# DonggeunYu/Text2Speech

Measured on AMD Instinct MI355X. Metric: WaveGlow forward audio samples/sec (batch 8x16000 per GPU), higher is better.
Workload: dtype bf16x3 (split-bf16 products, f32 accumulate); 1 GPU; WaveGlow forward, batch 8 x 16000 samples per GPU, 12 flows, n_group 8, WN 8 layers x 512 channels (reference waveglow/config.json); per_gpu_batch=8, segment_length=16000, mode=forward, parallelism=replicas, no collective

## Files before the change

include/t2s_hip.h:

```cpp
#ifndef T2S_HIP_H
#define T2S_HIP_H
#include <stddef.h>
#ifdef __cplusplus
extern "C" {
#endif

#define T2S_OK 0
#define T2S_EINVAL (-1)
#define T2S_EHIP (-2)

#define T2S_PERM_NONE 0
#define T2S_PERM_GATE 1
#define T2S_PERM_PAIR8 2
#define T2S_ACT_NONE 0
#define T2S_ACT_RELU 1
#define T2S_ACT_TANH 2

int t2s_abi_version(void);
int t2s_operand_format(void);
int t2s_sizeof_taco_decoder(void);
int t2s_sizeof_taco_bptt(void);
const char* t2s_error_string(int code);
const char* t2s_last_hip_error(void);

int t2s_plane_rows(int L, int halo);
int t2s_padded_rows(int rows);

int t2s_pack_conv_weight(const float* v, const float* g, int g_is_scale, const float* bias_in, int O, int Cin, int Kt,
                         int perm, int C_gate, int row_off, int Mpad, int koff, int Cin_pad, void* A_hi, void* A_lo,
                         float* bias_out, int bias_accumulate, void* stream);

typedef struct t2s_pack_job {
    const float *v, *g, *bias_in, *bias_in2;
    void *A_hi, *A_lo;
    float* bias_out;
    long row_start;
    long O, Cin, Kt, perm, C_gate, Mpad, koff, Cin_pad, row_off, g_is_scale;
    float* scale_out;
} t2s_pack_job;
int t2s_pack_conv_weight_table(const t2s_pack_job* jobs, int n_jobs, long total_groups, void* stream);

int t2s_weightnorm_small(const float* v, const float* g, int O, int K, float* w, void* stream);

int t2s_wg_upsample_squeeze(const float* mel, const float* W, const float* bias, int B, int n_mel, int frames,
                            int ksize, int stride, int n_group, int L, int Lp, int halo, void* S_hi, void* S_lo,
                            void* stream);

int t2s_wg_audio_squeeze(float* audio, float* z, int B, int T, int n_group, int L, int unsqueeze, void* stream);

int t2s_wg_convinv(float* z, const float* W, int B, int n_group, int c_off, int n_rem, int L, void* stream);

int t2s_small_logdet_inv(const float* W, int n, float scale, float* logdet_out, float* inv_out, void* stream);

typedef struct t2s_small_mat_job { const float* W; float* logdet_out; float* inv_out; long n; } t2s_small_mat_job;
int t2s_small_logdet_inv_batch(const t2s_small_mat_job* jobs, int n_jobs, float scale, void* stream);
int t2s_small_logdet_inv_batch_host(const t2s_small_mat_job* host_jobs, int n_jobs, float scale, void* stream);

int t2s_wg_start(const float* z, const float* w, const float* bias, int B, int n_group, int c_off, int n_half, int C,
                 int L, int Lp, int halo, void* X_hi, void* X_lo, void* stream);

int t2s_wg_in_cond_gate(const void* A_hi, const void* A_lo, const float* bias, const void* X_hi, const void* X_lo,
                        const void* S_hi, const void* S_lo, void* acts_hi, void* acts_lo, int B, int C, int n_cond,
                        int taps, int dilation, int L, int Lp, int halo, int Mpad, void* stream);

int t2s_wg_res_skip(const void* A_hi, const void* A_lo, const float* bias, const void* acts_hi, const void* acts_lo,
                    void* X_hi, void* X_lo, float* skip, int B, int C, int n_res, int skip_init, int L, int Lp,
                    int halo, int Mpad, void* stream);

int t2s_wg_end_affine(const float* skip, const float* w_end, const float* b_end, float* z, float* log_s,
                      float* wn_out, int B, int n_group, int c_off, int n_half, int C, int L, int Lp, int halo, int reverse, void* stream);

typedef struct t2s_endfold_job {
    const float *w_end, *v_skip, *scale, *b_skip;
    void* fold_A;
    float* bes;
    long nj, C;
} t2s_endfold_job;
int t2s_wg_endfold_weights(const t2s_endfold_job* jobs, int n_jobs, int C, void* stream);
int t2s_wg_gate_tile_rows(int B, int C, int L);
int t2s_wg_gate_fold_slots(int B, int C, int L);
int t2s_wg_in_cond_gate_fold(const void* A_hi, const void* A_lo, const float* bias, const void* X_hi, const void* X_lo,
                             const void* S_hi, const void* S_lo, void* acts_hi, void* acts_lo, const void* fold_A,
                             float* fold_acc, int fold_init, int B, int C, int n_cond, int taps, int dilation, int L,
                             int Lp, int halo, int Mpad, void* stream);
int t2s_wg_start_window(const float* z, const float* w, const float* bias, int B, int n_group, int c_off, int n_half, int C,
                        int L, int Lp, int halo, void* X_hi, void* X_lo, int taps, int win_chunks, void* W_hi, void* W_lo,
                        void* stream);
int t2s_wg_startfold_weights(const float* v_in, const float* g_in, const float* w_start, const float* b_start, int C, int n_half,
                             int taps, int Mpad, int win_chunks, void* A_hi, void* A_lo, void* stream);
int t2s_wg_in_win_gate_fold(const void* A_hi, const void* A_lo, const float* bias, const void* W_hi, const void* W_lo,
                            const void* S_hi, const void* S_lo, void* acts_hi, void* acts_lo, const void* fold_A,
                            float* fold_acc, int fold_init, int B, int C, int n_cond, int win_chunks, int L, int Lp, int halo,
                            int Mpad, void* stream);
int t2s_wg_upsample_basis(const float* W, const float* bias, int n_mel, int ksize, int stride, int n_group, int Lp, int halo,
                          void* U_hi, void* U_lo, void* stream);
int t2s_wg_compose_cond(const float* tmp, const float* bias_in, int rows, int Mpad, int P, int K2, long ld, void* A2_hi,
                        void* A2_lo, float* bias_out, void* stream);
int t2s_wg_melwin_planes(const float* mel, int B, int n_mel, int frames, int nlag, int Fp, void* M_hi, void* M_lo, void* stream);
int t2s_wg_in_melwin_gate_fold(const void* A_hi, const void* A_lo, const void* A2_hi, const void* A2_lo, const float* bias,
                               const void* X_hi, const void* X_lo, const void* M_hi, const void* M_lo, void* acts_hi,
                               void* acts_lo, const void* fold_A, float* fold_acc, int fold_init, int B, int C, int K2,
                               int taps, int dilation, int L, int Lp, int halo, int Mpad, int P, int Fp, void* stream);
int t2s_wg_res_only(const void* A_hi, const void* A_lo, const float* bias, const void* acts_hi, const void* acts_lo,
                    void* X_hi, void* X_lo, int B, int C, int L, int Lp, int halo, int Mpad, int pair8, void* stream);
int t2s_wg_res_only_start(const void* A_hi, const void* A_lo, const float* bias, const void* acts_hi, const void* acts_lo,
                          const float* z, const float* w_start, const float* b_start, int n_group, int c_off, int n_half,
                          void* X_hi, void* X_lo, int B, int C, int L, int Lp, int halo, int Mpad, void* stream);
int t2s_pack_conv_weight_table_h16(const t2s_pack_job* jobs, int n_jobs, long total_groups, void* stream);
int t2s_wg_endfold_weights_h16(const t2s_endfold_job* jobs, int n_jobs, int C, void* stream);
int t2s_wg_upsample_squeeze_h16(const float* mel, const float* W, const float* bias, int B, int n_mel, int frames,
                                int ksize, int stride, int n_group, int L, int Lp, int halo, void* S_hi, void* S_lo,
                                void* stream);
int t2s_wg_start_h16(const float* z, const float* w, const float* bias, int B, int n_group, int c_off, int n_half, int C,
                     int L, int Lp, int halo, void* X_hi, void* X_lo, void* stream);
int t2s_wg_in_cond_gate_fold_h16(const void* A_hi, const void* A_lo, const float* bias, const void* X_hi, const void* X_lo,
                                 const void* S_hi, const void* S_lo, void* acts_hi, void* acts_lo, const void* fold_A,
                                 float* fold_acc, int fold_init, int B, int C, int n_cond, int taps, int dilation, int L,
                                 int Lp, int halo, int Mpad, void* stream);
int t2s_wg_res_only_h16(const void* A_hi, const void* A_lo, const float* bias, const void* acts_hi, const void* acts_lo,
                        void* X_hi, void* X_lo, int B, int C, int L, int Lp, int halo, int Mpad, int pair8, void* stream);
int t2s_wg_flow_boundary(const float* z_in, float* z_out, const float* fold_acc, int nslots, const float* bes, int n_layers,
                         const float* b_end, float* log_s, int c_off_prev, int n_half_prev, const float* W, int c_off, int n_rem,
                         int n_half, int B, int n_group, int L, int Lp, int halo, int taps, int win_chunks, void* W_hi, void* W_lo,
                         void* stream);
int t2s_wg_start_ragged(const float* z, const float* w, const float* bias, int B, int n_group, int c_off, int n_half, int C,
                        int L, int Lp, int halo, void* X_hi, void* X_lo, int taps, int win_chunks, void* W_hi, void* W_lo,
                        const int* lengths, void* stream);
int t2s_wg_res_only_ragged(const void* A_hi, const void* A_lo, const float* bias, const void* acts_hi, const void* acts_lo,
                           void* X_hi, void* X_lo, int B, int C, int L, int Lp, int halo, int Mpad, int pair8, const int* lengths,
                           void* stream);
int t2s_wg_res_only_start_ragged(const void* A_hi, const void* A_lo, const float* bias, const void* acts_hi, const void* acts_lo,
                                 const float* z, const float* w_start, const float* b_start, int n_group, int c_off, int n_half,
                                 void* X_hi, void* X_lo, int B, int C, int L, int Lp, int halo, int Mpad, const int* lengths,
                                 void* stream);
int t2s_wg_flow_boundary_ragged(const float* z_in, float* z_out, const float* fold_acc, int nslots, const float* bes, int n_layers,
                                const float* b_end, float* log_s, int c_off_prev, int n_half_prev, const float* W, int c_off,
                                int n_rem, int n_half, int B, int n_group, int L, int Lp, int halo, int taps, int win_chunks,
                                void* W_hi, void* W_lo, const int* lengths, void* stream);
int t2s_wg_start_h16_ragged(const float* z, const float* w, const float* bias, int B, int n_group, int c_off, int n_half, int C,
                            int L, int Lp, int halo, void* X_hi, void* X_lo, const int* lengths, void* stream);
int t2s_wg_in_cond_gate_fold_h16_ragged(const void* A_hi, const void* A_lo, const float* bias, const void* X_hi, const void* X_lo,
                                        const void* S_hi, const void* S_lo, void* acts_hi, void* acts_lo, const void* fold_A,
                                        float* fold_acc, int fold_init, int B, int C, int n_cond, int taps, int dilation, int L,
                                        int Lp, int halo, int Mpad, const int* lengths, void* stream);
int t2s_wg_res_only_h16_ragged(const void* A_hi, const void* A_lo, const float* bias, const void* acts_hi, const void* acts_lo,
                               void* X_hi, void* X_lo, int B, int C, int L, int Lp, int halo, int Mpad, int pair8,
                               const int* lengths, void* stream);
int t2s_wg_end_fold_affine(const float* fold_acc, int nslots, const float* bes, int n_layers, const float* b_end,
                           float* z, float* log_s, float* wn_out, int B, int n_group, int c_off, int n_half, int L, int reverse,
                           void* stream);

int t2s_conv_bias_act(const void* A_hi, const void* A_lo, const float* bias, const void* X_hi, const void* X_lo,
                      void* O_hi, void* O_lo, float* out_f32, int f32_channel_last, int B, int Cin, int Cout, int taps,
                      int dilation, int act, int L, int Lp, int halo, int Mpad, void* stream);


int t2s_gemv(const float* W1, int ld1, int k1, const float* W2, int ld2, int k2, const float* x1, int n1, long sx1,
             const float* x2, int n2, long sx2, const float* x3, int n3, long sx3, const float* bias1,
             const float* bias2, float* y, long sy_item, long sy_row, int rows, int items, int act,
             const unsigned char* mask, long smask_item, float mask_scale, void* stream);

int t2s_transpose(const float* in, float* out, int R, int C, void* stream);

int t2s_embed_planes(const long* ids, const float* emb, int B, int T, int E, int V, int Lp, int halo, void* X_hi,
                     void* X_lo, void* stream);
int t2s_f32_to_planes(const float* x, int B, int C, int L, int Lp, int halo, void* X_hi, void* X_lo, void* stream);
int t2s_taco_parse_output(float* mel, float* mel_post, float* gate, const int* lengths, int B, int n_mel, int T, void* stream);
int t2s_zero_plane_rows(void* X_hi, void* X_lo, const int* lengths, int B, int C, int T, int Lp, int halo, void* stream);
int t2s_zero_rows_f32(float* x, const int* lengths, int B, int N, int row, void* stream);
int t2s_bn_fold(const float* gamma, const float* beta, const float* mean, const float* var, const float* conv_bias,
                float eps, int C, float* scale, float* bias_out, void* stream);

int t2s_bn_train(const float* x, const float* gamma, const float* beta, float eps, int act, const unsigned char* mask,
                 float mask_scale, int B, int C, int T, int Lp, int halo, float* mean, float* var, void* O_hi, void* O_lo,
                 float* out_f32, void* stream);

int t2s_bn_running_update(const float* mean, const float* var, float* running_mean, float* running_var,
                          long long* num_batches_tracked, float momentum, long long n, int C, void* stream);
int t2s_zero_fill(void* p, size_t bytes, void* stream);

int t2s_taco_encoder_lstm(const float* gx, const float* whhT_fwd, const float* whhT_rev, const int* lengths, float* out,
                          int B, int T, int H, int T_out, float* gates_save ,
                          float* c_save , void* stream);
int t2s_taco_encoder_lstm_split(const float* gx, const float* whhT_fwd, const float* whhT_rev, const int* lengths, float* out,
                                int B, int T, int H, int T_out, float* gates_save, float* c_save, void* xbuf, unsigned epoch,
                                void* stream);
long t2s_taco_lstm_xbuf_bytes(int B);
int t2s_taco_encoder_lstm_bwd(const float* d_out, const float* out, const float* gates_save, const float* c_save,
                              const float* whh_fwd, const float* whh_rev, const int* lengths, float* dgx, float* hprev,
                              int B, int T, int H, int T_out, void* stream);
int t2s_taco_encoder_lstm_bwd_split(const float* d_out, const float* out, const float* gates_save, const float* c_save,
                                    const float* whh_fwd, const float* whh_rev, const int* lengths, float* dgx, float* hprev,
                                    int B, int T, int H, int T_out, void* xbuf, unsigned epoch, void* stream);
int t2s_rows_to_planes(const float* x, int B, int T, int C, int Lp, int halo, void* X_hi, void* X_lo, void* stream);
int t2s_embedding_grad(const long* ids, const void* D_hi, const void* D_lo, int B, int T, int E, int V, int Lp, int halo,
                       float* d_emb, void* stream);

int t2s_bernoulli_mask(unsigned char* mask, size_t n, unsigned long long seed, unsigned long long offset, float keep_prob,
                       void* stream);

typedef struct t2s_taco_decoder {
    int B, T_in, n_mel, prenet_dim, enc_dim, att_rnn_dim, dec_rnn_dim, att_dim, loc_filters, loc_kernel;
    int T_cap;
    int teacher_forced;
    int mask_steps;
    const float *att_w_ih, *att_w_hh, *att_b_ih, *att_b_hh;
    const float *dec_w_ih, *dec_w_hh, *dec_b_ih, *dec_b_hh;
    const float *w_query, *w_loc_conv, *w_loc_dense, *w_v;
    const float *w_proj, *b_proj;
    const float *w_projpre, *b_projpre;
    const float *w_loc_denseT;
    const float *w_pre2;
    const float *memory, *pmem;
    const int *mem_lengths;
    const float *pre_all;
    const unsigned char *prenet_masks;
    const unsigned char *att_drop, *dec_drop;
    float att_drop_scale, dec_drop_scale;
    float *att_h0, *att_h1, *att_c, *dec_h0, *dec_h1, *dec_c;
    float *att_w, *att_wcum, *ctx, *q, *energies, *pre1, *pre2;
    float *q_part;
    float *mel_gate_out;
    float *align_out;
    float *hc_all;
    float *att_gates_all, *att_c_all;
    float *dec_gates_all, *dec_c_all;
    float *att_h_all;
    float *q_all, *wcum_all;
    float *gate_part;
    const float *w_pre2T;
    float *ploc;
    float *dec_in_part;
    void *att_xbuf;
    void *pace_flag;
} t2s_taco_decoder;

int t2s_taco_decode_steps(const t2s_taco_decoder* d, int step0, int n_steps, void* stream);

#define T2S_PLAN_SPLIT 0x001u
#define T2S_PLAN_PACED 0x002u
#define T2S_PLAN_SIG_BY_KERNEL 0x004u
#define T2S_PLAN_FUSED_ATT 0x008u
// ... 190 lines not shown
```

text2speech_amd/_lib.py:

```python
import ctypes
import os

HERE = os.path.dirname(os.path.abspath(__file__))
LIB_PATH = os.environ.get("T2S_LIB_PATH") or os.path.join(HERE, "libt2s_hip.so")

c_int, c_float, c_vp, c_long = ctypes.c_int, ctypes.c_float, ctypes.c_void_p, ctypes.c_long

SIGNATURES = {
    "t2s_abi_version": [],
    "t2s_operand_format": [],
    "t2s_sizeof_taco_decoder": [],
    "t2s_sizeof_taco_bptt": [],
    "t2s_error_string": [c_int],
    "t2s_last_hip_error": [],
    "t2s_plane_rows": [c_int, c_int],
    "t2s_padded_rows": [c_int],
    "t2s_pack_conv_weight": [c_vp, c_vp, c_int, c_vp, c_int, c_int, c_int, c_int, c_int, c_int, c_int, c_int, c_int,
                             c_vp, c_vp, c_vp, c_int, c_vp],
    "t2s_pack_conv_weight_table": [c_vp, c_int, c_long, c_vp],
    "t2s_weightnorm_small": [c_vp, c_vp, c_int, c_int, c_vp, c_vp],
    "t2s_wg_upsample_squeeze": [c_vp, c_vp, c_vp, c_int, c_int, c_int, c_int, c_int, c_int, c_int, c_int, c_int,
                                c_vp, c_vp, c_vp],
    "t2s_wg_audio_squeeze": [c_vp, c_vp, c_int, c_int, c_int, c_int, c_int, c_vp],
    "t2s_wg_convinv": [c_vp, c_vp, c_int, c_int, c_int, c_int, c_int, c_vp],
    "t2s_small_logdet_inv": [c_vp, c_int, c_float, c_vp, c_vp, c_vp],
    "t2s_small_logdet_inv_batch": [c_vp, c_int, c_float, c_vp],
    "t2s_small_logdet_inv_batch_host": [c_vp, c_int, c_float, c_vp],
    "t2s_wg_start": [c_vp, c_vp, c_vp, c_int, c_int, c_int, c_int, c_int, c_int, c_int, c_int, c_vp, c_vp, c_vp],
    "t2s_wg_in_cond_gate": [c_vp, c_vp, c_vp, c_vp, c_vp, c_vp, c_vp, c_vp, c_vp, c_int, c_int, c_int, c_int, c_int,
                            c_int, c_int, c_int, c_int, c_vp],
    "t2s_wg_res_skip": [c_vp, c_vp, c_vp, c_vp, c_vp, c_vp, c_vp, c_vp, c_int, c_int, c_int, c_int, c_int, c_int,
                        c_int, c_int, c_vp],
    "t2s_wg_endfold_weights": [c_vp, c_int, c_int, c_vp],
    "t2s_wg_in_cond_gate_fold": [c_vp] * 11 + [c_int] * 10 + [c_vp],
    "t2s_wg_start_window": [c_vp, c_vp, c_vp] + [c_int] * 8 + [c_vp, c_vp, c_int, c_int, c_vp, c_vp, c_vp],
    "t2s_wg_startfold_weights": [c_vp] * 4 + [c_int] * 5 + [c_vp, c_vp, c_vp],
    "t2s_wg_in_win_gate_fold": [c_vp] * 11 + [c_int] * 9 + [c_vp],
    "t2s_wg_gate_fold_slots": [c_int, c_int, c_int],
    "t2s_wg_gate_tile_rows": [c_int, c_int, c_int],
    "t2s_wg_upsample_basis": [c_vp, c_vp] + [c_int] * 6 + [c_vp, c_vp, c_vp],
    "t2s_wg_compose_cond": [c_vp, c_vp] + [c_int] * 4 + [c_long, c_vp, c_vp, c_vp, c_vp],
    "t2s_wg_melwin_planes": [c_vp] + [c_int] * 5 + [c_vp, c_vp, c_vp],
    "t2s_wg_in_melwin_gate_fold": [c_vp] * 13 + [c_int] * 12 + [c_vp],
    "t2s_wg_res_only": [c_vp] * 7 + [c_int] * 7 + [c_vp],
    "t2s_wg_res_only_start": [c_vp] * 8 + [c_int] * 3 + [c_vp, c_vp] + [c_int] * 6 + [c_vp],
    "t2s_wg_flow_boundary": [c_vp, c_vp, c_vp, c_int, c_vp, c_int, c_vp, c_vp, c_int, c_int, c_vp] + [c_int] * 10 + [c_vp, c_vp, c_vp],
    "t2s_wg_start_ragged": [c_vp, c_vp, c_vp] + [c_int] * 8 + [c_vp, c_vp, c_int, c_int, c_vp, c_vp, c_vp, c_vp],
    "t2s_wg_res_only_ragged": [c_vp] * 7 + [c_int] * 7 + [c_vp, c_vp],
    "t2s_wg_res_only_start_ragged": [c_vp] * 8 + [c_int] * 3 + [c_vp, c_vp] + [c_int] * 6 + [c_vp, c_vp],
    "t2s_wg_flow_boundary_ragged": [c_vp, c_vp, c_vp, c_int, c_vp, c_int, c_vp, c_vp, c_int, c_int, c_vp] + [c_int] * 10 + [c_vp, c_vp, c_vp, c_vp],
    "t2s_wg_end_fold_affine": [c_vp, c_int, c_vp, c_int, c_vp, c_vp, c_vp, c_vp, c_int, c_int, c_int, c_int, c_int, c_int, c_vp],
    "t2s_wg_end_affine": [c_vp, c_vp, c_vp, c_vp, c_vp, c_vp, c_int, c_int, c_int, c_int, c_int, c_int, c_int, c_int,
                          c_int, c_vp],
    "t2s_conv_bias_act": [c_vp, c_vp, c_vp, c_vp, c_vp, c_vp, c_vp, c_vp, c_int, c_int, c_int, c_int, c_int, c_int, c_int,
                          c_int, c_int, c_int, c_int, c_vp],
    "t2s_gemv": [c_vp, c_int, c_int, c_vp, c_int, c_int, c_vp, c_int, c_long, c_vp, c_int, c_long, c_vp, c_int, c_long,
                 c_vp, c_vp, c_vp, c_long, c_long, c_int, c_int, c_int, c_vp, c_long, c_float, c_vp],
    "t2s_transpose": [c_vp, c_vp, c_int, c_int, c_vp],
    "t2s_embed_planes": [c_vp, c_vp, c_int, c_int, c_int, c_int, c_int, c_int, c_vp, c_vp, c_vp],
    "t2s_f32_to_planes": [c_vp, c_int, c_int, c_int, c_int, c_int, c_vp, c_vp, c_vp],
    "t2s_taco_parse_output": [c_vp, c_vp, c_vp, c_vp, c_int, c_int, c_int, c_vp],
    "t2s_zero_plane_rows": [c_vp, c_vp, c_vp, c_int, c_int, c_int, c_int, c_int, c_vp],
    "t2s_zero_rows_f32": [c_vp, c_vp, c_int, c_int, c_int, c_vp],
    "t2s_bn_fold": [c_vp, c_vp, c_vp, c_vp, c_vp, c_float, c_int, c_vp, c_vp, c_vp],
    "t2s_bn_train": [c_vp, c_vp, c_vp, c_float, c_int, c_vp, c_float, c_int, c_int, c_int, c_int, c_int, c_vp, c_vp, c_vp,
                     c_vp, c_vp, c_vp],
    "t2s_taco_encoder_lstm": [c_vp, c_vp, c_vp, c_vp, c_vp, c_int, c_int, c_int, c_int, c_vp, c_vp, c_vp],
    "t2s_taco_encoder_lstm_bwd": [c_vp] * 9 + [c_int] * 4 + [c_vp],
    "t2s_taco_encoder_lstm_split": [c_vp, c_vp, c_vp, c_vp, c_vp, c_int, c_int, c_int, c_int, c_vp, c_vp, c_vp, ctypes.c_uint, c_vp],
    "t2s_taco_lstm_xbuf_bytes": [c_int],
    "t2s_taco_encoder_lstm_bwd_split": [c_vp] * 9 + [c_int] * 4 + [c_vp, ctypes.c_uint, c_vp],
    "t2s_rows_to_planes": [c_vp, c_int, c_int, c_int, c_int, c_int, c_vp, c_vp, c_vp],
    "t2s_embedding_grad": [c_vp, c_vp, c_vp, c_int, c_int, c_int, c_int, c_int, c_int, c_vp, c_vp],
    "t2s_bn_running_update": [c_vp, c_vp, c_vp, c_vp, c_vp, c_float, ctypes.c_longlong, c_int, c_vp],
    "t2s_zero_fill": [c_vp, ctypes.c_size_t, c_vp],
    "t2s_wg_bwd_pair8_ok": [c_int, c_int, c_int],
    "t2s_taco_attention": [c_vp] * 14 + [c_int] * 7 + [c_vp],
    "t2s_bernoulli_mask": [c_vp, ctypes.c_size_t, ctypes.c_ulonglong, ctypes.c_ulonglong, c_float, c_vp],
    "t2s_taco_decode_steps": [c_vp, c_int, c_int, c_vp],
    "t2s_taco_decode_plan": [c_vp, c_int, c_int, c_vp],
    "t2s_taco_decode_steps_w16": [c_vp, c_vp, c_int, c_int, c_vp],
    "t2s_taco_decode_plan_w16": [c_vp, c_vp, c_int, c_int, c_vp, c_vp],
    "t2s_taco_stop_check": [c_vp, c_int, c_int, c_int, c_int, c_int, c_float, c_vp, c_vp],
    "t2s_rows_to_tm": [c_vp, c_long, c_int, c_int, c_int, c_int, c_vp, c_vp, c_int, c_int, c_vp],
    "t2s_rows_to_tm_batched": [c_vp, c_long, c_long, c_int, c_int, c_int, c_int, c_vp, c_vp, c_long, c_int, c_int, c_int, c_vp],
    "t2s_lstm_cell_bwd": [c_vp, c_long, c_vp, c_long, c_vp, c_long, c_vp, c_float, c_vp, c_vp, c_vp, c_vp, c_vp, c_int, c_int,
                          c_vp],
    "t2s_relu_drop_bwd": [c_vp, c_vp, c_float, ctypes.c_size_t, c_vp, c_vp],
    "t2s_taco_att_bwd": [c_vp, c_vp],
    "t2s_taco_bptt_steps": [c_vp, c_int, c_int, c_vp],
    "t2s_bn_bwd": [c_vp, c_vp, c_vp],
    "t2s_waveglow_loss": [c_vp, ctypes.c_size_t, c_vp, c_vp, c_int, c_vp, c_float, c_vp, c_vp, c_vp, c_vp],
    "t2s_taco_loss": [c_vp, c_vp, c_vp, ctypes.c_size_t, c_vp, c_vp, ctypes.c_size_t, c_vp, c_vp, c_vp, c_vp, c_vp, c_vp],
    "t2s_stft_transform": [c_vp, c_int, c_int, c_vp, c_int, c_int, c_vp, c_long, c_vp, c_vp, c_vp, c_vp, c_long, c_vp],
    "t2s_mel_from_mag": [c_vp, c_long, c_int, c_int, c_vp, c_int, c_float, c_vp, c_vp],
    "t2s_stft_inverse": [c_vp, c_vp, c_int, c_int, c_int, c_int, c_vp, c_long, c_vp, c_float, c_vp, c_float, c_vp, c_vp, c_vp,
                         c_vp],
    "t2s_stft_transform_ragged": [c_vp, c_int, c_int, c_vp, c_vp, c_vp, c_int, c_int, c_vp, c_long, c_vp, c_vp, c_vp, c_vp, c_long,
                                  c_vp],
    "t2s_mel_from_mag_ragged": [c_vp, c_long, c_int, c_int, c_vp, c_vp, c_vp, c_int, c_float, c_vp, c_vp],
    "t2s_stft_inverse_ragged": [c_vp, c_vp, c_int, c_int, c_vp, c_vp, c_int, c_int, c_vp, c_long, c_vp, c_float, c_vp, c_float, c_vp,
                                c_vp, c_vp, c_vp],
    "t2s_pcm16": [c_vp, c_int, c_int, c_int, c_long, c_vp, c_vp, c_vp],
    "t2s_sum_axis0": [c_vp, c_int, c_int, c_vp, c_vp],
    "t2s_add3": [c_vp, c_vp, c_vp, ctypes.c_size_t, c_vp, c_vp],
    "t2s_scale_by_scalar": [c_vp, ctypes.c_size_t, c_vp, c_float, c_vp, c_vp],
    "t2s_planes_to_f32": [c_vp, c_vp, c_int, c_int, c_int, c_int, c_int, c_vp, c_int, c_vp],
    "t2s_wg_in_cond_gate_train": [c_vp] * 13 + [c_int] * 9 + [c_vp],
    "t2s_wg_res_skip_train": [c_vp] * 10 + [c_int] * 8 + [c_vp],
    "t2s_wg_bwd_gate_dgrad": [c_vp] * 11 + [c_int] + [c_vp] * 2 + [c_int] * 8 + [c_vp],
    "t2s_wg_in_cond_gate_fold_train": [c_vp] * 11 + [c_int] + [c_vp] * 2 + [c_int] * 10 + [c_vp],
    "t2s_wg_res_only_train": [c_vp] * 5 + [c_int] + [c_vp] * 4 + [c_int] * 7 + [c_vp],
    "t2s_wg_skip_sum": [c_vp] * 5 + [c_int] * 2 + [c_vp] + [c_int] * 6 + [c_vp],
    "t2s_conv_accumulate": [c_vp] * 5 + [c_int] + [c_vp] * 2 + [c_int] * 11 + [c_vp],
    "t2s_wgrad_gemm": [c_vp] * 6 + [c_int] * 9 + [c_vp],
    "t2s_wgrad_gemm_flat": [c_vp] * 6 + [c_int] * 9 + [c_vp],
    "t2s_wgrad_cl": [c_vp, c_int, c_vp, c_int, c_vp] + [c_int] * 8 + [c_vp],
    "t2s_plane_transpose": [c_vp, c_vp, c_int, c_int, c_int, c_int, c_int, c_vp, c_vp, c_int, c_int, c_vp],
    "t2s_tm_ones_row": [c_vp, c_vp, c_int, c_int, c_int, c_int, c_int, c_int, c_vp],
    "t2s_pack_transposed": [c_vp, c_vp, c_int, c_int, c_int, c_int, c_int, c_int, c_int, c_vp, c_vp, c_int, c_vp],
    "t2s_weightnorm_scale": [c_vp, c_vp, c_int, c_int, c_vp, c_vp],
    "t2s_wn_backward": [c_vp, c_int, c_int, c_int, c_int, c_int, c_int, c_int, c_int, c_vp, c_vp, c_int, c_int, c_int, c_vp, c_vp,
                        c_vp, c_int, c_vp],
    "t2s_wg_affine_backward": [c_vp, c_vp, c_vp, c_vp, c_int, c_vp, c_int, c_int, c_int, c_int, c_int, c_vp],
    "t2s_small_wgrad_scratch": [c_int, c_int],
    "t2s_small_wgrad": [c_vp, c_vp, c_vp, c_vp, c_vp, c_vp, c_vp, c_int, c_int, c_int, c_int, c_int, c_int, c_int, c_int, c_int,
                        c_int, c_vp],
    "t2s_rows_sum": [c_vp, c_int, c_int, c_int, c_int, c_int, c_vp, c_vp],
    "t2s_wg_start_dgrad": [c_vp, c_vp, c_vp, c_vp, c_int, c_int, c_int, c_int, c_int, c_int, c_int, c_int, c_vp],
    "t2s_wg_convinv_wgrad": [c_vp, c_vp, c_vp, c_vp, c_float, c_int, c_int, c_int, c_int, c_int, c_vp, c_vp],
    "t2s_wg_upsample_wgrad": [c_vp, c_vp, c_vp, c_int, c_int, c_int, c_int, c_int, c_int, c_int, c_int, c_int, c_vp, c_vp,
                              c_vp],
    "t2s_adam_table": [c_vp, c_int, c_long, c_float, c_float, c_float, c_float, c_int, c_float, c_float, c_vp],
}
for _n in ("t2s_pack_conv_weight_table", "t2s_wg_endfold_weights", "t2s_wg_upsample_squeeze", "t2s_wg_start",
           "t2s_wg_in_cond_gate_fold", "t2s_wg_res_only"):
    SIGNATURES[_n + "_h16"] = list(SIGNATURES[_n])
for _n in ("t2s_wg_start", "t2s_wg_in_cond_gate_fold", "t2s_wg_res_only"):
    SIGNATURES[_n + "_h16_ragged"] = SIGNATURES[_n + "_h16"][:-1] + [c_vp, c_vp]
del _n
_RESTYPE = {"t2s_error_string": ctypes.c_char_p, "t2s_last_hip_error": ctypes.c_char_p,
            "t2s_small_wgrad_scratch": ctypes.c_long, "t2s_taco_lstm_xbuf_bytes": ctypes.c_long}


class T2SError(RuntimeError):
    pass


class TacoW16(ctypes.Structure):
    _fields_ = [(n, c_vp) for n in ("att_w_ih", "att_w_hh", "dec_w_ih", "dec_w_hh")]


_lib = None


def load():
    global _lib
    if _lib is not None:
        return _lib
    if not os.path.exists(LIB_PATH):
        raise T2SError(
            "libt2s_hip.so not found at %s - build it with `python -m text2speech_amd.build` "
            "(there is no CPU fallback on the product path)" % LIB_PATH)
    lib = ctypes.CDLL(LIB_PATH)
    diagnostic = bool(os.environ.get("T2S_LIB_PATH"))
    for name, argtypes in SIGNATURES.items():
        try:
            fn = getattr(lib, name)
        except AttributeError as e:
            if diagnostic:
                continue
            raise T2SError("libt2s_hip.so does not export %s" % name) from e
        fn.argtypes = argtypes
        fn.restype = _RESTYPE.get(name, c_int)
    _lib = lib
    return lib


def ptr(t):
    if t is None:
        return None
    return c_vp(t.data_ptr())


HOST_TIMES = {}
_HOST_TIMING = bool(os.environ.get("T2S_HOST_TIMING"))


def call(name, *args):
# ... 37 lines not shown
```

text2speech_amd/csrc/t2s_api.hip:

```cpp
#include "../../include/t2s_hip.h"
#include "t2s_kernels.h"
#include "t2s_api_common.h"
#include "conv_gemm_args.h"

#include <stdlib.h>
#include <string.h>

static thread_local char g_hip_err[256] = "";

extern "C" int t2s_internal_fail_hip(int ei) {
    hipError_t e = (hipError_t)ei;
    strncpy(g_hip_err, hipGetErrorString(e), sizeof(g_hip_err) - 1);
    g_hip_err[sizeof(g_hip_err) - 1] = 0;
    return T2S_EHIP;
}


static inline bool a_operand_ok(const void* A_hi, const void* A_lo, bool h16) { return h16 ? (A_hi && al16(A_hi)) : planes_ok(A_hi, A_lo); }

static int pack_table(const t2s_pack_job* jobs, int n_jobs, long total_rows, void* stream, bool h16) {
    if (!jobs || n_jobs <= 0 || total_rows <= 0 || total_rows > 0x7fffffffL) return T2S_EINVAL;
    static_assert(sizeof(t2s_pack_job) == sizeof(PackJob), "t2s_pack_job layout");
    T2S_CHECK_HIP(t2s_launch_pack_table((const PackJob*)jobs, n_jobs, total_rows, (hipStream_t)stream, h16));
    return T2S_OK;
// ... 60 lines not shown
#else
    return 0;
#endif
}

const char* t2s_error_string(int code) {
    switch (code) {
        case T2S_OK: return "ok";
        case T2S_EINVAL: return "invalid argument";
        case T2S_EHIP: return "HIP runtime error";
        default: return "unknown error";
    }
}
const char* t2s_last_hip_error(void) { return g_hip_err; }

int t2s_plane_rows(int L, int halo) { return cdiv(L, 256) * 256 + 2 * halo; }
int t2s_padded_rows(int rows) { return cdiv(rows, 256) * 256; }

int t2s_pack_conv_weight(const float* v, const float* g, int g_is_scale, const float* bias_in, int O, int Cin, int Kt,
                         int perm, int C_gate, int row_off, int Mpad, int koff, int Cin_pad, void* A_hi, void* A_lo,
                         float* bias_out, int bias_accumulate, void* stream) {
    if (!v || !A_hi || !A_lo || O <= 0 || Cin <= 0 || Kt <= 0) return T2S_EINVAL;
    if (Mpad % 256 || koff % 32 || Cin_pad % 32 || Cin_pad < Cin) return T2S_EINVAL;
    if (perm == T2S_PERM_GATE) {
        if (O != 2 * C_gate || cdiv(C_gate, 128) * 256 > Mpad) return T2S_EINVAL;
    } else if (perm == T2S_PERM_NONE) {
        if (row_off < 0 || row_off + O > Mpad) return T2S_EINVAL;
    } else {
        return T2S_EINVAL;
    }
    PackArgs a;
    a.v = v; a.g = g; a.bias_in = bias_in;
    a.A_hi = (u16*)A_hi; a.A_lo = (u16*)A_lo; a.bias_out = bias_out;
    a.O = O; a.Cin = Cin; a.Kt = Kt; a.perm = perm; a.C_gate = C_gate; a.Mpad = Mpad; a.koff = koff;
    a.Cin_pad = Cin_pad; a.bias_accumulate = bias_accumulate; a.row_off = row_off; a.g_is_scale = g_is_scale;
    T2S_CHECK_HIP(t2s_launch_pack(a, (hipStream_t)stream));
    return T2S_OK;
}

int t2s_pack_conv_weight_table(const t2s_pack_job* jobs, int n_jobs, long total_rows, void* stream) {
    return pack_table(jobs, n_jobs, total_rows, stream, false);
}
int t2s_pack_conv_weight_table_h16(const t2s_pack_job* jobs, int n_jobs, long total_rows, void* stream) {
    return pack_table(jobs, n_jobs, total_rows, stream, true);
}

int t2s_weightnorm_small(const float* v, const float* g, int O, int K, float* w, void* stream) {
    if (!v || !w || O <= 0 || K <= 0) return T2S_EINVAL;
    T2S_CHECK_HIP(t2s_launch_weightnorm_small(v, g, O, K, w, (hipStream_t)stream));
    return T2S_OK;
}

int t2s_wg_upsample_squeeze(const float* mel, const float* W, const float* bias, int B, int n_mel, int frames,
                            int ksize, int stride, int n_group, int L, int Lp, int halo, void* S_hi, void* S_lo,
                            void* stream) {
    return upsample_squeeze(mel, W, bias, B, n_mel, frames, ksize, stride, n_group, L, Lp, halo, S_hi, S_lo, stream, false);
}
int t2s_wg_upsample_squeeze_h16(const float* mel, const float* W, const float* bias, int B, int n_mel, int frames,
                                int ksize, int stride, int n_group, int L, int Lp, int halo, void* S_hi, void* S_lo,
                                void* stream) {
    return upsample_squeeze(mel, W, bias, B, n_mel, frames, ksize, stride, n_group, L, Lp, halo, S_hi, S_lo, stream, true);
}

int t2s_wg_audio_squeeze(float* audio, float* z, int B, int T, int n_group, int L, int unsqueeze, void* stream) {
    if (!audio || !z || B <= 0 || L <= 0 || n_group <= 0 || (long)L * n_group > T) return T2S_EINVAL;
    T2S_CHECK_HIP(t2s_launch_audio_squeeze(audio, z, B, T, n_group, L, unsqueeze, (hipStream_t)stream));
    return T2S_OK;
}

int t2s_wg_convinv(float* z, const float* W, int B, int n_group, int c_off, int n_rem, int L, void* stream) {
    if (!z || !W || B <= 0 || L <= 0 || n_rem <= 0 || n_rem > 16 || c_off < 0 || c_off + n_rem > n_group) return T2S_EINVAL;
    T2S_CHECK_HIP(t2s_launch_convinv(z, W, B, n_group, c_off, n_rem, L, (hipStream_t)stream));
    return T2S_OK;
}

int t2s_small_logdet_inv(const float* W, int n, float scale, float* logdet_out, float* inv_out, void* stream) {
    if (!W || n <= 0 || n > 16 || (!logdet_out && !inv_out)) return T2S_EINVAL;
    T2S_CHECK_HIP(t2s_launch_small_logdet_inv(W, n, scale, logdet_out, inv_out, (hipStream_t)stream));
    return T2S_OK;
}

int t2s_small_logdet_inv_batch(const t2s_small_mat_job* jobs, int n_jobs, float scale, void* stream) {
    if (!jobs || n_jobs <= 0) return T2S_EINVAL;
    static_assert(sizeof(t2s_small_mat_job) == sizeof(SmallMatJob), "t2s_small_mat_job layout");
    T2S_CHECK_HIP(t2s_launch_small_logdet_batch((const SmallMatJob*)jobs, n_jobs, scale, (hipStream_t)stream));
    return T2S_OK;
}

int t2s_small_logdet_inv_batch_host(const t2s_small_mat_job* host_jobs, int n_jobs, float scale, void* stream) {
    if (!host_jobs || n_jobs <= 0 || n_jobs > 16) return T2S_EINVAL;
    for (int i = 0; i < n_jobs; ++i)
        if (!host_jobs[i].W || host_jobs[i].n <= 0 || host_jobs[i].n > 16) return T2S_EINVAL;
    T2S_CHECK_HIP(t2s_launch_small_logdet_batch_host((const SmallMatJob*)host_jobs, n_jobs, scale, (hipStream_t)stream));
    return T2S_OK;
}

int t2s_wg_start(const float* z, const float* w, const float* bias, int B, int n_group, int c_off, int n_half, int C,
                 int L, int Lp, int halo, void* X_hi, void* X_lo, void* stream) {
    return wg_start(z, w, bias, B, n_group, c_off, n_half, C, L, Lp, halo, X_hi, X_lo, stream, false);
}
int t2s_wg_start_h16(const float* z, const float* w, const float* bias, int B, int n_group, int c_off, int n_half, int C,
                     int L, int Lp, int halo, void* X_hi, void* X_lo, void* stream) {
    return wg_start(z, w, bias, B, n_group, c_off, n_half, C, L, Lp, halo, X_hi, X_lo, stream, true);
}
int t2s_wg_start_h16_ragged(const float* z, const float* w, const float* bias, int B, int n_group, int c_off, int n_half, int C,
                            int L, int Lp, int halo, void* X_hi, void* X_lo, const int* lengths, void* stream) {
    if (!lengths) return T2S_EINVAL;
    return wg_start(z, w, bias, B, n_group, c_off, n_half, C, L, Lp, halo, X_hi, X_lo, stream, true, lengths);
}

static bool win_chunks_ok(int taps, int n_half, int win_chunks) {
    if (taps <= 0 || !(taps & 1) || n_half <= 0 || (win_chunks != 2 && win_chunks != 4)) return false;
    return (4 / win_chunks) * taps * (n_half + 1) <= 32;
}

static int start_window(const float* z, const float* w, const float* bias, int B, int n_group, int c_off, int n_half, int C, int L,
                        int Lp, int halo, void* X_hi, void* X_lo, int taps, int win_chunks, void* W_hi, void* W_lo,
                        const int* lengths, void* stream) {
    if (!z || !w || !bias || !planes_ok(X_hi, X_lo) || !planes_ok(W_hi, W_lo)) return T2S_EINVAL;
    if (B <= 0 || L <= 0 || C <= 0 || n_half <= 0 || n_half > 8 || c_off < 0 || c_off + n_half > n_group) return T2S_EINVAL;
    if (!win_chunks_ok(taps, n_half, win_chunks) || cdiv(C, 32) < win_chunks || Lp < t2s_plane_rows(L, halo)) return T2S_EINVAL;
    T2S_CHECK_HIP(t2s_launch_start(z, w, bias, B, n_group, c_off, n_half, C, L, Lp, halo, (u16*)X_hi, (u16*)X_lo,
                                   (hipStream_t)stream, taps, win_chunks, (u16*)W_hi, (u16*)W_lo, lengths));
    return T2S_OK;
}

int t2s_wg_start_window(const float* z, const float* w, const float* bias, int B, int n_group, int c_off, int n_half, int C,
                        int L, int Lp, int halo, void* X_hi, void* X_lo, int taps, int win_chunks, void* W_hi, void* W_lo,
                        void* stream) {
    return start_window(z, w, bias, B, n_group, c_off, n_half, C, L, Lp, halo, X_hi, X_lo, taps, win_chunks, W_hi, W_lo, nullptr, stream);
}

int t2s_wg_start_ragged(const float* z, const float* w, const float* bias, int B, int n_group, int c_off, int n_half, int C,
                        int L, int Lp, int halo, void* X_hi, void* X_lo, int taps, int win_chunks, void* W_hi, void* W_lo,
                        const int* lengths, void* stream) {
    if (!lengths) return T2S_EINVAL;
    if (W_hi || W_lo)
        return start_window(z, w, bias, B, n_group, c_off, n_half, C, L, Lp, halo, X_hi, X_lo, taps, win_chunks, W_hi, W_lo, lengths, stream);
    if (!z || !w || !bias || !X_hi || !X_lo) return T2S_EINVAL;
    if (B <= 0 || L <= 0 || C <= 0 || n_half <= 0 || n_half > 8 || c_off < 0 || c_off + n_half > n_group) return T2S_EINVAL;
    if (!al16(X_hi) || !al16(X_lo) || Lp < t2s_plane_rows(L, halo)) return T2S_EINVAL;
    T2S_CHECK_HIP(t2s_launch_start(z, w, bias, B, n_group, c_off, n_half, C, L, Lp, halo, (u16*)X_hi, (u16*)X_lo,
                                   (hipStream_t)stream, 0, 0, nullptr, nullptr, lengths));
    return T2S_OK;
}

int t2s_wg_startfold_weights(const float* v_in, const float* g_in, const float* w_start, const float* b_start, int C, int n_half,
                             int taps, int Mpad, int win_chunks, void* A_hi, void* A_lo, void* stream) {
    if (!v_in || !w_start || !b_start || !planes_ok(A_hi, A_lo)) return T2S_EINVAL;
    if (C <= 0 || !win_chunks_ok(taps, n_half, win_chunks)) return T2S_EINVAL;
    if (Mpad % 256 || Mpad < cdiv(C, 128) * 256 || (size_t)C * (n_half + 1) * sizeof(float) > 60 * 1024) return T2S_EINVAL;
    T2S_CHECK_HIP(t2s_launch_startfold_weights(v_in, g_in, w_start, b_start, C, n_half, taps, Mpad, win_chunks, (u16*)A_hi, (u16*)A_lo,
                                               (hipStream_t)stream));
    return T2S_OK;
}

int t2s_wg_in_cond_gate(const void* A_hi, const void* A_lo, const float* bias, const void* X_hi, const void* X_lo,
                        const void* S_hi, const void* S_lo, void* acts_hi, void* acts_lo, int B, int C, int n_cond,
                        int taps, int dilation, int L, int Lp, int halo, int Mpad, void* stream) {
    if (!planes_ok(A_hi, A_lo) || !planes_ok(X_hi, X_lo) || !planes_ok(acts_hi, acts_lo) || !bias || !al16(bias)) return T2S_EINVAL;
    if ((n_cond > 0 && !planes_ok(S_hi, S_lo)) || !gate_shape_ok(B, C, taps, dilation, L, Lp, halo, Mpad)) return T2S_EINVAL;
    ConvGemm g(A_hi, A_lo, bias);
    g.geometry(B, L, Lp, halo, Mpad);
    g.k_side(X_hi, X_lo, cdiv(C, 32), taps, dilation, S_hi, S_lo, cdiv(n_cond, 32));
    g.output(acts_hi, acts_lo, cdiv(C, 32));
    g.a.C = C;
    T2S_CHECK_HIP(g.launch(EPI_GATE, 2 * C, 256, stream));
    return T2S_OK;
}

int t2s_wg_res_skip(const void* A_hi, const void* A_lo, const float* bias, const void* acts_hi, const void* acts_lo,
                    void* X_hi, void* X_lo, float* skip, int B, int C, int n_res, int skip_init, int L, int Lp,
                    int halo, int Mpad, void* stream) {
    if (!planes_ok(A_hi, A_lo) || !planes_ok(acts_hi, acts_lo) || !bias || !al16(bias) || !skip || !al16(skip)) return T2S_EINVAL;
    if (n_res > 0 && !planes_ok(X_hi, X_lo)) return T2S_EINVAL;
    if (C <= 0 || C % 4 || (n_res != 0 && n_res != C) || !geometry_ok(B, L, Lp, halo, Mpad, n_res + C)) return T2S_EINVAL;
    ConvGemm g(A_hi, A_lo, bias);
    g.geometry(B, L, Lp, halo, Mpad);
    g.k_side(acts_hi, acts_lo, cdiv(C, 32), 1, 1);
    g.output(X_hi, X_lo, cdiv(C, 32));
    g.a.skip = skip; g.a.C = C; g.a.n_res = n_res; g.a.skip_init = skip_init;
    T2S_CHECK_HIP(g.launch(EPI_RESSKIP, n_res + C, 256, stream));
    return T2S_OK;
}

int t2s_wg_endfold_weights(const t2s_endfold_job* jobs, int n_jobs, int C, void* stream) {
    return endfold_weights(jobs, n_jobs, C, stream, false);
}
int t2s_wg_endfold_weights_h16(const t2s_endfold_job* jobs, int n_jobs, int C, void* stream) {
    return endfold_weights(jobs, n_jobs, C, stream, true);
}

int t2s_wg_gate_tile_rows(int B, int C, int L) {
    if (B <= 0 || C <= 0 || L <= 0) return T2S_EINVAL;
    return gate_tile_rows(B, C, L);
}

int t2s_wg_gate_fold_slots(int B, int C, int L) {
    if (B <= 0 || C <= 0 || L <= 0) return T2S_EINVAL;
    return gate_tile_rows(B, C, L) == 128 ? 2 * cdiv(C, 64) : 2 * cdiv(C, 128);
}

int t2s_wg_in_cond_gate_fold(const void* A_hi, const void* A_lo, const float* bias, const void* X_hi, const void* X_lo,
                             const void* S_hi, const void* S_lo, void* acts_hi, void* acts_lo, const void* fold_A,
                             float* fold_acc, int fold_init, int B, int C, int n_cond, int taps, int dilation, int L,
                             int Lp, int halo, int Mpad, void* stream) {
    return in_cond_gate_fold(A_hi, A_lo, bias, X_hi, X_lo, S_hi, S_lo, acts_hi, acts_lo, fold_A, fold_acc, fold_init, B, C, n_cond, taps,
                             dilation, L, Lp, halo, Mpad, stream, false);
}
int t2s_wg_in_cond_gate_fold_h16(const void* A_hi, const void* A_lo, const float* bias, const void* X_hi, const void* X_lo,
                                 const void* S_hi, const void* S_lo, void* acts_hi, void* acts_lo, const void* fold_A,
                                 float* fold_acc, int fold_init, int B, int C, int n_cond, int taps, int dilation, int L,
                                 int Lp, int halo, int Mpad, void* stream) {
    return in_cond_gate_fold(A_hi, A_lo, bias, X_hi, X_lo, S_hi, S_lo, acts_hi, acts_lo, fold_A, fold_acc, fold_init, B, C, n_cond, taps,
                             dilation, L, Lp, halo, Mpad, stream, true);
}
int t2s_wg_in_cond_gate_fold_h16_ragged(const void* A_hi, const void* A_lo, const float* bias, const void* X_hi, const void* X_lo,
                                        const void* S_hi, const void* S_lo, void* acts_hi, void* acts_lo, const void* fold_A,
                                        float* fold_acc, int fold_init, int B, int C, int n_cond, int taps, int dilation, int L,
                                        int Lp, int halo, int Mpad, const int* lengths, void* stream) {
    if (!lengths) return T2S_EINVAL;
    return in_cond_gate_fold(A_hi, A_lo, bias, X_hi, X_lo, S_hi, S_lo, acts_hi, acts_lo, fold_A, fold_acc, fold_init, B, C, n_cond, taps,
                             dilation, L, Lp, halo, Mpad, stream, true, lengths);
}

int t2s_wg_in_win_gate_fold(const void* A_hi, const void* A_lo, const float* bias, const void* W_hi, const void* W_lo,
                            const void* S_hi, const void* S_lo, void* acts_hi, void* acts_lo, const void* fold_A,
                            float* fold_acc, int fold_init, int B, int C, int n_cond, int win_chunks, int L, int Lp, int halo,
                            int Mpad, void* stream) {
    if (!planes_ok(A_hi, A_lo) || !planes_ok(W_hi, W_lo) || !planes_ok(S_hi, S_lo) || !planes_ok(acts_hi, acts_lo) || !bias ||
        !al16(bias))
        return T2S_EINVAL;
    if (!fold_ok(fold_A, fold_acc, C) || C <= 0 || n_cond <= 0 || halo < 0 || (win_chunks != 2 && win_chunks != 4)) return T2S_EINVAL;
    if (!geometry_ok(B, L, Lp, halo, Mpad, cdiv(C, 128) * 256)) return T2S_EINVAL;
    ConvGemm g(A_hi, A_lo, bias);
    g.geometry(B, L, Lp, halo, Mpad);
    g.k_side(W_hi, W_lo, win_chunks, 1, 1, S_hi, S_lo, cdiv(n_cond, 32));
    g.output(acts_hi, acts_lo, cdiv(C, 32));
    g.fold(fold_A, fold_acc, fold_init);
    g.a.C = C;
    T2S_CHECK_HIP(g.launch(EPI_GATE, 2 * C, gate_tile_rows(B, C, L), stream));
    return T2S_OK;
}

int t2s_wg_upsample_basis(const float* W, const float* bias, int n_mel, int ksize, int stride, int n_group, int Lp, int halo,
                          void* U_hi, void* U_lo, void* stream) {
    if (!W || !bias || !planes_ok(U_hi, U_lo)) return T2S_EINVAL;
    if (n_mel <= 0 || n_group <= 0 || stride <= 0 || ksize <= 0 || ksize % stride || stride % n_group) return T2S_EINVAL;
    const int ncols = (stride / n_group) * (ksize / stride) * n_mel + 1;
    if (halo < 0 || Lp != t2s_plane_rows(ncols, halo)) return T2S_EINVAL;
    T2S_CHECK_HIP(t2s_launch_upbasis_planes(W, bias, n_mel, ksize, stride, n_group, Lp, halo, (u16*)U_hi, (u16*)U_lo,
                                            (hipStream_t)stream));
    return T2S_OK;
}

int t2s_wg_compose_cond(const float* tmp, const float* bias_in, int rows, int Mpad, int P, int K2, long ld, void* A2_hi,
                        void* A2_lo, float* bias_out, void* stream) {
    if (!tmp || !bias_in || !bias_out || !planes_ok(A2_hi, A2_lo)) return T2S_EINVAL;
    if (rows <= 0 || Mpad % 256 || rows > Mpad || P <= 0 || K2 <= 0 || K2 % 32 || ld < (long)P * K2 + 1) return T2S_EINVAL;
    T2S_CHECK_HIP(t2s_launch_compose_pack(tmp, bias_in, rows, Mpad, P, K2, (int)ld, (u16*)A2_hi, (u16*)A2_lo, bias_out,
                                          (hipStream_t)stream));
    return T2S_OK;
}

int t2s_wg_melwin_planes(const float* mel, int B, int n_mel, int frames, int nlag, int Fp, void* M_hi, void* M_lo, void* stream) {
    if (!mel || !planes_ok(M_hi, M_lo)) return T2S_EINVAL;
    if (B <= 0 || n_mel <= 0 || frames <= 0 || nlag <= 0 || Fp < frames) return T2S_EINVAL;
    T2S_CHECK_HIP(t2s_launch_melwin_planes(mel, B, n_mel, frames, nlag, Fp, (u16*)M_hi, (u16*)M_lo, (hipStream_t)stream));
    return T2S_OK;
}

int t2s_wg_in_melwin_gate_fold(const void* A_hi, const void* A_lo, const void* A2_hi, const void* A2_lo, const float* bias,
                               const void* X_hi, const void* X_lo, const void* M_hi, const void* M_lo, void* acts_hi,
                               void* acts_lo, const void* fold_A, float* fold_acc, int fold_init, int B, int C, int K2,
                               int taps, int dilation, int L, int Lp, int halo, int Mpad, int P, int Fp, void* stream) {
    if (!planes_ok(A_hi, A_lo) || !planes_ok(A2_hi, A2_lo) || !planes_ok(X_hi, X_lo) || !planes_ok(M_hi, M_lo) ||
        !planes_ok(acts_hi, acts_lo) || !bias || !al16(bias))
        return T2S_EINVAL;
    if (!fold_ok(fold_A, fold_acc, C) || !gate_shape_ok(B, C, taps, dilation, L, Lp, halo, Mpad)) return T2S_EINVAL;
    if (K2 <= 0 || K2 % 32 || P <= 0) return T2S_EINVAL;
    const int F = cdiv(L, P);
    if (Fp < F || gate_tile_rows(B, C, L) != 256) return T2S_EINVAL;
    ConvGemm g(A_hi, A_lo, bias);
    g.geometry(B, L, Lp, halo, Mpad);
    g.k_side(X_hi, X_lo, cdiv(C, 32), taps, dilation, M_hi, M_lo, K2 / 32);
    g.output(acts_hi, acts_lo, cdiv(C, 32));
    g.fold(fold_A, fold_acc, fold_init);
    g.a.A2_hi = (const u16*)A2_hi; g.a.A2_lo = (const u16*)A2_lo;
    g.a.C = C;
    g.a.n_ttiles = 0;
    g.a.ph_P = P; g.a.ph_Fp = Fp;
    g.a.ph_FT = F <= 64 ? 64 : (F <= 128 ? 128 : 256);
    g.a.ph_bper = 256 / g.a.ph_FT;
    g.a.ph_nft = cdiv(F, g.a.ph_FT);
    T2S_CHECK_HIP(g.launch(EPI_GATE, 2 * C, 256, stream));
    return T2S_OK;
}

static int res_only(const void* A_hi, const void* A_lo, const float* bias, const void* acts_hi, const void* acts_lo,
                    void* X_hi, void* X_lo, int B, int C, int L, int Lp, int halo, int Mpad, int pair8, const int* lengths,
                    void* stream, bool h16 = false) {
    if (!a_operand_ok(A_hi, A_lo, h16) || !planes_ok(acts_hi, acts_lo) || !planes_ok(X_hi, X_lo) || !bias || !al16(bias)) return T2S_EINVAL;
    if (C <= 0 || C % 4 || (pair8 && C % 32) || !geometry_ok(B, L, Lp, halo, Mpad, C)) return T2S_EINVAL;
    ConvGemm g(A_hi, A_lo, bias);
    g.geometry(B, L, Lp, halo, Mpad);
    g.k_side(acts_hi, acts_lo, cdiv(C, 32), 1, 1);
// ... 145 lines not shown
```

text2speech_amd/csrc/t2s_kernels.h:

```cpp
#pragma once
#include <hip/hip_runtime.h>
#include <stdint.h>

typedef unsigned short u16;

enum { EPI_GATE = 0, EPI_RESSKIP = 1, EPI_BIAS_ACT = 2, EPI_GATE_BWD = 3 };
enum { ACT_NONE = 0, ACT_RELU = 1, ACT_TANH = 2 };
enum { PERM_NONE = 0, PERM_GATE = 1, PERM_PAIR8 = 2 };

struct ConvGemmArgs {
    const u16* A_hi;
    const u16* A_lo;
    const u16* X_hi;
    const u16* X_lo;
    const u16* S_hi;
    const u16* S_lo;
    const float* bias;
    u16* O_hi;
    u16* O_lo;
    float* skip;
    float* out_f32;
    int nk;
    int nk_x;
    int xc, sc, oc;
    int xbs;
    int taps, dil;
    int Mpad, Lp, halo, L, B;
    int n_mtiles, n_ttiles;
    int C;
    int n_res;
    int skip_init;
    int act;
    int f32_cl;
    u16* T_hi;
    u16* T_lo;
    u16* G_hi;
    u16* G_lo;
    int tc;
    int pair8;
    int res_init;
    const u16* R_hi;
    const u16* R_lo;
    long a_bstride;
    int ksplit;
    int k0, kchunk, kend;
    int kflat;
    const u16* fold_A;
    float* fold_acc;
    int fold_init;
    const u16* A2_hi;
    const u16* A2_lo;
    int ph_P;
    int ph_FT;
    int ph_bper;
    int ph_nft;
    int ph_Fp;
    const float* x0_z;
    const float* x0_w;
    const float* x0_b;
    int x0_G, x0_coff, x0_nh;
    const int* lengths;
};

#define T2S_RAG_SKIP_COLS 256
#ifdef __HIPCC__
static __device__ __forceinline__ void t2s_rag_zero_fold(const ConvGemmArgs& a, int mt, int b, int t0, int tid) {
    if (!a.fold_A || !a.fold_init) return;
    const int ncols = min(T2S_RAG_SKIP_COLS, a.L - t0);
    for (int idx = tid; idx < 16 * T2S_RAG_SKIP_COLS; idx += 512) {
        const int col = idx % T2S_RAG_SKIP_COLS, sj = idx / T2S_RAG_SKIP_COLS;
        if (col < ncols) a.fold_acc[(((size_t)(mt * 2 + (sj >> 3)) * a.B + b) * 8 + (sj & 7)) * a.L + t0 + col] = 0.f;
    }
}
#endif

hipError_t t2s_launch_conv_gemm(const ConvGemmArgs& a, int epi, hipStream_t stream, int mt_rows = 256, bool h16 = false);
hipError_t t2s_launch_gate_gemm_pp(const ConvGemmArgs& a, hipStream_t stream, bool h16 = false);
hipError_t t2s_launch_bwd_gemm_pp(const ConvGemmArgs& a, int epi, hipStream_t stream);
bool t2s_pp_shape_ok(const ConvGemmArgs& a);

struct WgradChunk {
    const u16* hi;
    const u16* lo;
    long bstride;
};
struct WgradClArgs {
    const WgradChunk* a_chunks;
    const WgradChunk* b_chunks;
    float* P;
    int M, N, ldp, n_mtiles, n_ntiles;
    int B, k0, k1;
    int nslab, kchunk;
    int bias_cols;
};
hipError_t t2s_launch_wgrad_cl(const WgradClArgs& a, hipStream_t stream);

struct PackArgs {
    const float* v;
    const float* g;
    const float* bias_in;
    u16* A_hi;
    u16* A_lo;
    float* bias_out;
    int O, Cin, Kt;
    int perm, C_gate;
    int Mpad;
    int koff;
    int Cin_pad;
    int bias_accumulate;
    int row_off;
    int g_is_scale;
};
hipError_t t2s_launch_pack(const PackArgs& a, hipStream_t stream);
struct PackJob {
    const float* v; const float* g; const float* bias_in; const float* bias_in2;
    u16* A_hi; u16* A_lo; float* bias_out;
    long row_start;
    long O, Cin, Kt, perm, C_gate, Mpad, koff, Cin_pad, row_off, g_is_scale;
    float* scale_out;
};
hipError_t t2s_launch_pack_table(const PackJob* jobs, int n_jobs, long total_rows, hipStream_t stream, bool h16 = false);
hipError_t t2s_launch_weightnorm_small(const float* v, const float* g, int O, int K, float* w, hipStream_t stream);

hipError_t t2s_launch_upbasis_planes(const float* W, const float* bias, int n_mel, int ksize, int stride, int n_group, int Lp,
                                     int halo, u16* U_hi, u16* U_lo, hipStream_t stream);
hipError_t t2s_launch_compose_pack(const float* tmp, const float* bias_in, int rows, int Mpad, int P, int K2, int ld, u16* A2_hi,
                                   u16* A2_lo, float* bias_out, hipStream_t stream);
hipError_t t2s_launch_melwin_planes(const float* mel, int B, int n_mel, int frames, int nlag, int Fp, u16* S_hi, u16* S_lo,
                                    hipStream_t stream);
hipError_t t2s_launch_upsample_squeeze(const float* mel, const float* W, const float* bias, int B, int n_mel,
                                       int frames, int ksize, int stride, int n_group, int L, int Lp, int halo,
                                       u16* S_hi, u16* S_lo, hipStream_t stream, bool h16 = false);
hipError_t t2s_launch_audio_squeeze(const float* audio, float* z, int B, int T, int n_group, int L, int unsqueeze,
                                    hipStream_t stream);
hipError_t t2s_launch_convinv(float* z, const float* W, int B, int n_group, int c_off, int n_rem, int L,
                              hipStream_t stream);
struct SmallMatJob { const float* W; float* logdet_out; float* inv_out; long n; };
hipError_t t2s_launch_small_logdet_batch(const SmallMatJob* jobs, int n_jobs, float scale, hipStream_t stream);
hipError_t t2s_launch_small_logdet_batch_host(const SmallMatJob* host_jobs, int n_jobs, float scale, hipStream_t stream);
hipError_t t2s_launch_small_logdet_inv(const float* W, int n, float scale, float* logdet_out, float* inv_out,
                                       hipStream_t stream);
hipError_t t2s_launch_start(const float* z, const float* w, const float* bias, int B, int n_group, int c_off,
                            int n_half, int C, int L, int Lp, int halo, u16* X_hi, u16* X_lo, hipStream_t stream,
                            int taps = 0, int nwc = 0, u16* W_hi = nullptr, u16* W_lo = nullptr, const int* lengths = nullptr,
                            bool h16 = false);
hipError_t t2s_launch_startfold_weights(const float* v, const float* g, const float* w_start, const float* b_start, int C,
                                        int n_half, int taps, int Mpad, int nwc, u16* A_hi, u16* A_lo, hipStream_t stream);
struct EndFoldJob {
    const float* w_end;
    const float* v_skip;
    const float* scale;
    const float* b_skip;
    u16* fold_A;
    float* bes;
    long nj, C;
};
hipError_t t2s_launch_endfold_weights(const EndFoldJob* jobs, int n_jobs, int C, hipStream_t stream, bool h16 = false);
hipError_t t2s_launch_end_fold_affine(const float* fold_acc, int nslots, const float* bes, int n_layers,
                                      const float* b_end, float* z, float* log_s, float* wn_out, int B, int n_group, int c_off,
                                      int n_half, int L, int reverse, hipStream_t stream);
struct FlowBoundaryArgs {
    const float* z_in;
    float* z_out;
    const float* fold_acc;
    const float* bes;
    const float* b_end;
    float* log_s;
    const float* W;
    u16* W_hi;
    u16* W_lo;
    int nslots, n_layers, c_off_prev, nh_prev;
    int c_off, n_rem, nh;
    int G, L, Lp, halo, taps, nwc;
    const int* lengths;
};
hipError_t t2s_launch_flow_boundary(const FlowBoundaryArgs& a, int B, hipStream_t stream);
int t2s_flow_boundary_max_taps();
hipError_t t2s_launch_end_affine(const float* skip, const float* w_end, const float* b_end, float* z, float* log_s,
                                 float* wn_out, int B, int n_group, int c_off, int n_half, int C, int L, int Lp, int halo,
                                 int reverse, hipStream_t stream);
```

text2speech_amd/csrc/waveglow_ops.hip:

```cpp
#include "t2s_common.h"
#include "t2s_kernels.h"

#include <string.h>

static __device__ __forceinline__ void pack_row(const float* __restrict__ vrow, const float* g, int g_is_scale, int o,
                                                 int Cin, int Kt, int perm, int C_gate, int row_off, int Mpad, int koff,
                                                 int Cin_pad, u16* A_hi, u16* A_lo, const float* bias_in,
                                                 const float* bias_in2, float* bias_out, int bias_accumulate,
                                                 float* scale_out = nullptr) {
    __shared__ float red[4];
    const int tid = threadIdx.x;
    const int n = Cin * Kt;
    float scale = 1.0f;
    if (g && g_is_scale) {
        scale = g[o];
    } else if (g) {
        float ss = 0.f;
        for (int i = tid; i < n; i += 256) {
            const float x = vrow[i];
            ss += x * x;
        }
        ss = wave_sum(ss);
        if ((tid & 63) == 0) red[tid >> 6] = ss;
        __syncthreads();
        ss = red[0] + red[1] + red[2] + red[3];
        scale = g[o] / sqrtf(ss);
    }
    if (scale_out && tid == 0) scale_out[o] = scale;
    int p;
    if (perm == PERM_GATE) {
        const int gate = o >= C_gate;
        const int ch = gate ? o - C_gate : o;
        p = (ch >> 7) * 256 + ((ch >> 6) & 1) * 128 + (((ch >> 4) & 3) * 2 + gate) * 16 + (ch & 15);
    } else {
        p = o + row_off;
    }
    const int half = (Cin + 1) >> 1;
    for (int i = tid; i < half * Kt; i += 256) {
        const int tap = i / half;
        const int c = (i - tap * half) * 2;
        const float w0 = vrow[c * Kt + tap] * scale;
        const float w1 = (c + 1 < Cin) ? vrow[(c + 1) * Kt + tap] * scale : 0.f;
        const int k = koff + tap * Cin_pad + c;
        const size_t idx = ((size_t)(k >> 5) * Mpad + p) * 32 + (k & 31);
        u16 h0, l0, h1, l1;
        split_bf16(w0, h0, l0);
        split_bf16(w1, h1, l1);
        *(uint32_t*)(A_hi + idx) = h0 | ((uint32_t)h1 << 16);
        *(uint32_t*)(A_lo + idx) = l0 | ((uint32_t)l1 << 16);
    }
    if (tid == 0 && bias_out) {
        float bi = bias_in ? bias_in[o] : 0.f;
        if (bias_in2) bi += bias_in2[o];
        bias_out[p] = bias_accumulate ? bias_out[p] + bi : bi;
    }
}

__global__ __launch_bounds__(256) void pack_kernel(const PackArgs a) {
    const int o = blockIdx.x;
    pack_row(a.v + (size_t)o * a.Cin * a.Kt, a.g, a.g_is_scale, o, a.Cin, a.Kt, a.perm, a.C_gate, a.row_off, a.Mpad,
             a.koff, a.Cin_pad, a.A_hi, a.A_lo, a.bias_in, nullptr, a.bias_out, a.bias_accumulate);
}

static __device__ __forceinline__ int pack_dst_row(const PackJob& j, int o) {
    if (j.perm == PERM_GATE) {
        const int gate = o >= (int)j.C_gate;
        const int ch = gate ? o - (int)j.C_gate : o;
        return (ch >> 7) * 256 + ((ch >> 6) & 1) * 128 + (((ch >> 4) & 3) * 2 + gate) * 16 + (ch & 15);
    }
    if (j.perm == PERM_PAIR8 && o < (int)j.C_gate) {
        const int w = o & 31;
        return (o & ~31) + ((w >> 2) & 1) * 16 + (w >> 3) * 4 + (w & 3) + (int)j.row_off;
    }
    return o + (int)j.row_off;
}
template <class FMT, bool ONE>
static __device__ __forceinline__ void pack_store2(const PackJob& j, int k, int p, float w0, float w1) {
    const size_t idx = ((size_t)(k >> 5) * (int)j.Mpad + p) * 32 + (k & 31);
    u16 h0, l0, h1, l1;
    split_fmt<FMT>(w0, h0, l0);
    split_fmt<FMT>(w1, h1, l1);
    *(uint32_t*)(j.A_hi + idx) = h0 | ((uint32_t)h1 << 16);
    if constexpr (!ONE) *(uint32_t*)(j.A_lo + idx) = l0 | ((uint32_t)l1 << 16);
}
static __device__ __forceinline__ float sum16(float v) {
    v += __shfl_xor(v, 1, 64); v += __shfl_xor(v, 2, 64); v += __shfl_xor(v, 4, 64); v += __shfl_xor(v, 8, 64);
    return v;
}
#define PACK_MAX_CHUNKS 20
template <int KT, class FMT, bool ONE>
static __device__ __forceinline__ void pack_rows_regs(const PackJob& j, int o0) {
    const int tid = threadIdx.x, r = tid >> 4, cp = tid & 15;
    const int O = (int)j.O, Cin = (int)j.Cin, Cin_pad = (int)j.Cin_pad, koff = (int)j.koff;
    const int o = o0 + r;
    const bool row_ok = o < O;
    const int n = Cin * KT;
    const int nchunk = (Cin + 31) >> 5;
    const float* vrow = j.v + (size_t)(row_ok ? o : 0) * n;
    float x[PACK_MAX_CHUNKS][2 * KT];
    float ss = 0.f;
#pragma unroll
    for (int cc = 0; cc < PACK_MAX_CHUNKS; ++cc) {
        const int c = cc * 32 + cp * 2;
#pragma unroll
        for (int e = 0; e < 2 * KT; ++e) {
            const int ce = c + e / KT;
            x[cc][e] = (cc < nchunk && row_ok && ce < Cin) ? vrow[c * KT + e] : 0.f;
            ss += x[cc][e] * x[cc][e];
        }
    }
    float scale = 1.0f;
    if (j.g) {
        if (j.g_is_scale) scale = row_ok ? j.g[o] : 1.f;
        else {
            ss = sum16(ss);
            scale = row_ok ? j.g[o] / sqrtf(ss) : 1.f;
        }
    }
    if (!row_ok) return;
    const int p = pack_dst_row(j, o);
    if (cp == 0) {
        if (j.scale_out) j.scale_out[o] = scale;
        if (j.bias_out) {
            float bi = j.bias_in ? j.bias_in[o] : 0.f;
            if (j.bias_in2) bi += j.bias_in2[o];
            j.bias_out[p] = bi;
        }
    }
#pragma unroll
    for (int cc = 0; cc < PACK_MAX_CHUNKS; ++cc) {
        if (cc < nchunk) {
            const int c = cc * 32 + cp * 2;
#pragma unroll
            for (int tap = 0; tap < KT; ++tap)
                pack_store2<FMT, ONE>(j, koff + tap * Cin_pad + c, p, x[cc][tap] * scale, x[cc][KT + tap] * scale);
        }
    }
}

template <class FMT, bool ONE>
static __device__ __forceinline__ void pack_rows_two_pass(const PackJob& j, int o0, float* s_scale) {
    const int tid = threadIdx.x, lane = tid & 63, wave = tid >> 6;
    const int O = (int)j.O, Cin = (int)j.Cin, Kt = (int)j.Kt, Cin_pad = (int)j.Cin_pad, koff = (int)j.koff;
    const int n = Cin * Kt;
#pragma unroll
    for (int rr = 0; rr < 4; ++rr) {
        const int r = wave * 4 + rr, o = o0 + r;
        float scale = 1.0f;
        if (o < O && j.g) {
            if (j.g_is_scale) {
                scale = j.g[o];
            } else {
                const float* vrow = j.v + (size_t)o * n;
                float ss = 0.f;
                for (int i = lane; i < n; i += 64) {
                    const float x = vrow[i];
                    ss += x * x;
                }
                ss = wave_sum(ss);
                scale = j.g[o] / sqrtf(ss);
            }
        }
        if (lane == 0) {
            s_scale[r] = scale;
            if (o < O) {
                if (j.scale_out) j.scale_out[o] = scale;
                if (j.bias_out) {
                    float bi = j.bias_in ? j.bias_in[o] : 0.f;
                    if (j.bias_in2) bi += j.bias_in2[o];
                    j.bias_out[pack_dst_row(j, o)] = bi;
                }
            }
        }
    }
    __syncthreads();
    const int r = tid >> 4, cp = tid & 15;
    const int o = o0 + r;
    if (o >= O) return;
    const int p = pack_dst_row(j, o);
    const float scale = s_scale[r];
    const float* vrow = j.v + (size_t)o * n;
    const int nchunk = (Cin + 31) >> 5;
    for (int cc = 0; cc < nchunk; ++cc) {
        const int c = cc * 32 + cp * 2;
        for (int tap = 0; tap < Kt; ++tap) {
            const float w0 = c < Cin ? vrow[c * Kt + tap] * scale : 0.f;
            const float w1 = c + 1 < Cin ? vrow[(c + 1) * Kt + tap] * scale : 0.f;
            pack_store2<FMT, ONE>(j, koff + tap * Cin_pad + c, p, w0, w1);
        }
    }
}

template <class FMT = T2sFmt, bool ONE = false>
__global__ __launch_bounds__(256) void pack_table_kernel(const PackJob* __restrict__ jobs, int n_jobs) {
    __shared__ float s_scale[16];
    const long blk = blockIdx.x;
    int lo = 0, hi = n_jobs - 1;
    while (lo < hi) {
        const int mid = (lo + hi + 1) >> 1;
        if (jobs[mid].row_start <= blk) lo = mid; else hi = mid - 1;
    }
    const PackJob j = jobs[lo];
    const int o0 = (int)(blk - j.row_start) * 16;
    const int nchunk = ((int)j.Cin + 31) >> 5;
    if (nchunk <= PACK_MAX_CHUNKS && !((int)j.Cin & 1) && j.Kt == 3) pack_rows_regs<3, FMT, ONE>(j, o0);
    else if (nchunk <= PACK_MAX_CHUNKS && !((int)j.Cin & 1) && j.Kt == 1) pack_rows_regs<1, FMT, ONE>(j, o0);
    else pack_rows_two_pass<FMT, ONE>(j, o0, s_scale);
}
hipError_t t2s_launch_pack_table(const PackJob* jobs, int n_jobs, long total_groups, hipStream_t stream, bool h16) {
    if (h16) hipLaunchKernelGGL((pack_table_kernel<T2sFmtF16, true>), dim3((unsigned)total_groups), dim3(256), 0, stream, jobs, n_jobs);
    else hipLaunchKernelGGL((pack_table_kernel<>), dim3((unsigned)total_groups), dim3(256), 0, stream, jobs, n_jobs);
    return hipGetLastError();
}

hipError_t t2s_launch_pack(const PackArgs& a, hipStream_t stream) {
    hipLaunchKernelGGL(pack_kernel, dim3(a.O), dim3(256), 0, stream, a);
    return hipGetLastError();
}

__global__ void weightnorm_small_kernel(const float* v, const float* g, int O, int K, float* w) {
    const int o = blockIdx.x * blockDim.x + threadIdx.x;
    if (o >= O) return;
    float ss = 0.f;
    for (int k = 0; k < K; ++k) ss += v[o * K + k] * v[o * K + k];
    const float s = g ? g[o] / sqrtf(ss) : 1.f;
    for (int k = 0; k < K; ++k) w[o * K + k] = v[o * K + k] * s;
}
hipError_t t2s_launch_weightnorm_small(const float* v, const float* g, int O, int K, float* w, hipStream_t stream) {
    hipLaunchKernelGGL(weightnorm_small_kernel, dim3((O + 255) / 256), dim3(256), 0, stream, v, g, O, K, w);
    return hipGetLastError();
}

template <int BB, class FMT = T2sFmt>
__global__ __launch_bounds__(256) void upsample_squeeze_kernel(const float* __restrict__ mel, const float* __restrict__ W,
                                                               const float* __restrict__ bias, int B, int M, int F,
                                                               int ksize, int stride, int G, int L, int Lp, int halo,
                                                               u16* S_hi, u16* S_lo) {
    const int tid = threadIdx.x;
    const int q = tid & 3;
    const int t = blockIdx.x * 64 + (tid >> 2);
    const int chunk = blockIdx.y;
    const int b0 = blockIdx.z * BB;
    const int c8 = chunk * 32 + q * 8;
    const int nchan = M * G;
    if (t >= L || c8 >= nchan) return;
    float acc[BB][8];
#pragma unroll
    for (int bb = 0; bb < BB; ++bb)
#pragma unroll
        for (int j = 0; j < 8; ++j) acc[bb][j] = 0.f;
    const int nf = ksize / stride;
    if (G == 8) {
        const int co = c8 >> 3;
        const int s0 = 8 * t;
        const int fhi = s0 / stride;
        const int kbase = s0 - fhi * stride;
        for (int ci = 0; ci < M; ++ci) {
            const float* wrow = W + ((size_t)ci * M + co) * ksize + kbase;
            for (int i = 0; i < nf; ++i) {
                const int f = fhi - i;
                if (f < 0 || f >= F) continue;
                const f32x4 w0 = *(const f32x4*)(wrow + i * stride);
                const f32x4 w1 = *(const f32x4*)(wrow + i * stride + 4);
#pragma unroll
                for (int bb = 0; bb < BB; ++bb) {
                    if (b0 + bb >= B) break;
                    const float m = mel[((size_t)(b0 + bb) * M + ci) * F + f];
#pragma unroll
                    for (int j = 0; j < 4; ++j) {
                        acc[bb][j] += m * w0[j];
                        acc[bb][4 + j] += m * w1[j];
                    }
                }
            }
        }
#pragma unroll
        for (int bb = 0; bb < BB; ++bb)
#pragma unroll
            for (int j = 0; j < 8; ++j) acc[bb][j] += bias[co];
    } else {
        for (int j = 0; j < 8; ++j) {
            const int cidx = c8 + j;
            if (cidx >= nchan) break;
            const int co = cidx / G, g = cidx - co * G;
            const int s = G * t + g;
            const int fhi = s / stride;
            for (int ci = 0; ci < M; ++ci)
                for (int i = 0; i < nf; ++i) {
                    const int f = fhi - i;
                    if (f < 0 || f >= F) continue;
                    const float w = W[((size_t)ci * M + co) * ksize + (s - f * stride)];
                    for (int bb = 0; bb < BB; ++bb)
                        if (b0 + bb < B) acc[bb][j] += mel[((size_t)(b0 + bb) * M + ci) * F + f] * w;
                }
            for (int bb = 0; bb < BB; ++bb) acc[bb][j] += bias[co];
        }
    }
    const int nchunks = (nchan + 31) / 32;
#pragma unroll
    for (int bb = 0; bb < BB; ++bb) {
        if (b0 + bb >= B) break;
        const size_t row = ((size_t)(b0 + bb) * nchunks + chunk) * Lp + halo + t;
        u16 hi[8], lo[8];
#pragma unroll
        for (int j = 0; j < 8; ++j) {
            const float v = (c8 + j < nchan) ? acc[bb][j] : 0.f;
            split_fmt<FMT>(v, hi[j], lo[j]);
        }
        uint4 ph, pl;
        ph.x = hi[0] | ((uint32_t)hi[1] << 16); ph.y = hi[2] | ((uint32_t)hi[3] << 16);
        ph.z = hi[4] | ((uint32_t)hi[5] << 16); ph.w = hi[6] | ((uint32_t)hi[7] << 16);
        pl.x = lo[0] | ((uint32_t)lo[1] << 16); pl.y = lo[2] | ((uint32_t)lo[3] << 16);
        pl.z = lo[4] | ((uint32_t)lo[5] << 16); pl.w = lo[6] | ((uint32_t)lo[7] << 16);
        *(uint4*)(S_hi + row * 32 + q * 8) = ph;
        *(uint4*)(S_lo + row * 32 + q * 8) = pl;
    }
}

typedef float f32x4_up __attribute__((ext_vector_type(4)));
template <int NT, int KB, class FMT = T2sFmt>
__global__ __launch_bounds__(256) void upsample_mfma_kernel(const float* __restrict__ mel, const float* __restrict__ W,
                                                            const float* __restrict__ bias, int B, int M, int F, int ksize,
                                                            int stride, int L, int Lp, int halo, int tiles_per_b, int n_ctiles,
                                                            int n_pairs, int nz, u16* S_hi, u16* S_lo) {
    const int lane = threadIdx.x & 63;
    const int wave = threadIdx.x >> 6;
    const int r = lane & 15, q = lane >> 4;
    const int xcd = blockIdx.x & 7, slot = blockIdx.x >> 3;
    const int pair = (slot / nz) * 8 + xcd;
    if (pair >= n_pairs) return;
    const int npb = stride >> 6;
    const int p0 = ((pair % npb) * 4 + wave) * 16;
    const int chunk = pair / npb;
    const int ct0 = (slot % nz) * NT;
    const float* wa = W + (size_t)(chunk * 4) * ksize + (size_t)q * stride + p0 + r;
    const size_t wa_step = (size_t)M * ksize;
    const float* mb[NT];
    bool mv[NT];
#pragma unroll
    for (int n = 0; n < NT; ++n) {
        const int ct = ct0 + n;
        const int b = ct / tiles_per_b;
        const int f = (ct - b * tiles_per_b) * 16 + r - q;
        mv[n] = ct < n_ctiles && b < B && f >= 0 && f < F;
        mb[n] = mel + ((size_t)(mv[n] ? b : 0) * M) * F + (mv[n] ? f : 0);
    }
    f32x4_up acc[4][NT];
#pragma unroll
    for (int o = 0; o < 4; ++o)
#pragma unroll
        for (int n = 0; n < NT; ++n) acc[o][n] = (f32x4_up){0.f, 0.f, 0.f, 0.f};
    float a_cur[KB][4], b_cur[KB][NT], a_nxt[KB][4], b_nxt[KB][NT];
#pragma unroll
    for (int kk = 0; kk < KB; ++kk) {
#pragma unroll
        for (int o = 0; o < 4; ++o) a_cur[kk][o] = wa[(size_t)kk * wa_step + (size_t)o * ksize];
#pragma unroll
        for (int n = 0; n < NT; ++n) b_cur[kk][n] = mv[n] ? mb[n][(size_t)kk * F] : 0.f;
    }
    for (int ci = 0; ci < M; ci += KB) {
// ... 116 lines not shown
                                     int halo, u16* U_hi, u16* U_lo, hipStream_t stream) {
    const int P = stride / n_group, K2 = (ksize / stride) * n_mel;
    const int ncols = P * K2 + 1;
    dim3 grid((ncols + 63) / 64, (n_mel * n_group + 31) / 32);
    hipLaunchKernelGGL(upbasis_planes_kernel, grid, dim3(256), 0, stream, W, bias, n_mel, ksize, stride, n_group, P, K2, Lp, halo,
                       U_hi, U_lo);
    return hipGetLastError();
}

__global__ __launch_bounds__(256) void compose_pack_kernel(const float* __restrict__ tmp, const float* __restrict__ bias_in,
                                                           int rows, int Mpad, int P, int K2, int ld, u16* A2_hi, u16* A2_lo,
                                                           float* bias_out) {
    const int q = threadIdx.x & 3;
    const int m = blockIdx.x * 64 + (threadIdx.x >> 2);
    const int kc = blockIdx.y, phi = blockIdx.z;
    if (m >= Mpad) return;
    u16 hi[8], lo[8];
#pragma unroll
    for (int e = 0; e < 8; ++e) {
        const int k = kc * 32 + q * 8 + e;
        const float v = (m < rows && k < K2) ? tmp[(size_t)m * ld + (size_t)phi * K2 + k] : 0.f;
        split_bf16(v, hi[e], lo[e]);
    }
    const int mc = (K2 + 31) / 32;
    const size_t o = ((((size_t)phi * mc + kc) * Mpad) + m) * 32 + q * 8;
    uint4 ph, pl;
    ph.x = hi[0] | ((uint32_t)hi[1] << 16); ph.y = hi[2] | ((uint32_t)hi[3] << 16);
    ph.z = hi[4] | ((uint32_t)hi[5] << 16); ph.w = hi[6] | ((uint32_t)hi[7] << 16);
    pl.x = lo[0] | ((uint32_t)lo[1] << 16); pl.y = lo[2] | ((uint32_t)lo[3] << 16);
    pl.z = lo[4] | ((uint32_t)lo[5] << 16); pl.w = lo[6] | ((uint32_t)lo[7] << 16);
    *(uint4*)(A2_hi + o) = ph;
    *(uint4*)(A2_lo + o) = pl;
    if (kc == 0 && phi == 0 && q == 0) bias_out[m] = bias_in[m] + (m < rows ? tmp[(size_t)m * ld + (size_t)P * K2] : 0.f);
}
hipError_t t2s_launch_compose_pack(const float* tmp, const float* bias_in, int rows, int Mpad, int P, int K2, int ld, u16* A2_hi,
                                   u16* A2_lo, float* bias_out, hipStream_t stream) {
    dim3 grid((Mpad + 63) / 64, (K2 + 31) / 32, P);
    hipLaunchKernelGGL(compose_pack_kernel, grid, dim3(256), 0, stream, tmp, bias_in, rows, Mpad, P, K2, ld, A2_hi, A2_lo, bias_out);
    return hipGetLastError();
}

__global__ __launch_bounds__(256) void melwin_planes_kernel(const float* __restrict__ mel, int M, int F, int nlag, int Fp,
                                                            u16* S_hi, u16* S_lo) {
    const int q = threadIdx.x & 3;
    const int f = blockIdx.x * 64 + (threadIdx.x >> 2);
    const int chunk = blockIdx.y, b = blockIdx.z;
    if (f >= Fp) return;
    const int K2 = nlag * M, mc = (K2 + 31) / 32;
    u16 hi[8], lo[8];
#pragma unroll
    for (int e = 0; e < 8; ++e) {
        const int k = chunk * 32 + q * 8 + e;
        float v = 0.f;
        if (k < K2) {
            const int j = k / M, ci = k - j * M;
            const int ff = f - j;
            if (ff >= 0 && ff < F) v = mel[((size_t)b * M + ci) * F + ff];
        }
        split_bf16(v, hi[e], lo[e]);
    }
    const size_t o = (((size_t)b * mc + chunk) * Fp + f) * 32 + q * 8;
    uint4 ph, pl;
    ph.x = hi[0] | ((uint32_t)hi[1] << 16); ph.y = hi[2] | ((uint32_t)hi[3] << 16);
    ph.z = hi[4] | ((uint32_t)hi[5] << 16); ph.w = hi[6] | ((uint32_t)hi[7] << 16);
    pl.x = lo[0] | ((uint32_t)lo[1] << 16); pl.y = lo[2] | ((uint32_t)lo[3] << 16);
    pl.z = lo[4] | ((uint32_t)lo[5] << 16); pl.w = lo[6] | ((uint32_t)lo[7] << 16);
    *(uint4*)(S_hi + o) = ph;
    *(uint4*)(S_lo + o) = pl;
}
hipError_t t2s_launch_melwin_planes(const float* mel, int B, int n_mel, int frames, int nlag, int Fp, u16* S_hi, u16* S_lo,
                                    hipStream_t stream) {
    dim3 grid((Fp + 63) / 64, (nlag * n_mel + 31) / 32, B);
    hipLaunchKernelGGL(melwin_planes_kernel, grid, dim3(256), 0, stream, mel, n_mel, frames, nlag, Fp, S_hi, S_lo);
    return hipGetLastError();
}

__global__ void audio_squeeze_kernel(const float* audio, float* z, int B, int T, int G, int L, int unsq) {
    const int t = blockIdx.x * blockDim.x + threadIdx.x;
    const int b = blockIdx.y;
    if (t >= L) return;
    for (int g = 0; g < G; ++g) {
        if (unsq)
            ((float*)audio)[(size_t)b * T + (size_t)G * t + g] = z[((size_t)b * G + g) * L + t];
        else
            z[((size_t)b * G + g) * L + t] = audio[(size_t)b * T + (size_t)G * t + g];
    }
}
hipError_t t2s_launch_audio_squeeze(const float* audio, float* z, int B, int T, int n_group, int L, int unsqueeze,
                                    hipStream_t stream) {
    hipLaunchKernelGGL(audio_squeeze_kernel, dim3((L + 255) / 256, B), dim3(256), 0, stream, audio, z, B, T, n_group,
                       L, unsqueeze);
    return hipGetLastError();
}

__global__ void convinv_kernel(float* z, const float* __restrict__ W, int G, int c_off, int n, int L) {
    __shared__ float w[16 * 16];
    if (threadIdx.x < n * n) w[threadIdx.x] = W[threadIdx.x];
    __syncthreads();
    const int t = blockIdx.x * blockDim.x + threadIdx.x;
    const int b = blockIdx.y;
    if (t >= L) return;
    float* base = z + ((size_t)b * G + c_off) * L + t;
    float v[16], o[16];
    for (int j = 0; j < n; ++j) v[j] = base[(size_t)j * L];
    for (int i = 0; i < n; ++i) {
        float s = 0.f;
        for (int j = 0; j < n; ++j) s += w[i * n + j] * v[j];
        o[i] = s;
    }
    for (int i = 0; i < n; ++i) base[(size_t)i * L] = o[i];
}
hipError_t t2s_launch_convinv(float* z, const float* W, int B, int n_group, int c_off, int n_rem, int L,
                              hipStream_t stream) {
    hipLaunchKernelGGL(convinv_kernel, dim3((L + 255) / 256, B), dim3(256), 0, stream, z, W, n_group, c_off, n_rem, L);
    return hipGetLastError();
}

__global__ void small_logdet_inv_kernel(const float* W, int n, float scale, float* logdet_out, float* inv_out) {
    __shared__ double a[16][32];
    if (threadIdx.x != 0 || blockIdx.x != 0) return;
    for (int i = 0; i < n; ++i)
        for (int j = 0; j < n; ++j) {
            a[i][j] = W[i * n + j];
            a[i][n + j] = (i == j) ? 1.0 : 0.0;
        }
    double logabs = 0.0;
    int sign = 1;
    for (int c = 0; c < n; ++c) {
        int piv = c;
        double best = fabs(a[c][c]);
        for (int r = c + 1; r < n; ++r)
            if (fabs(a[r][c]) > best) { best = fabs(a[r][c]); piv = r; }
        if (piv != c) {
            for (int j = 0; j < 2 * n; ++j) { double tmp = a[c][j]; a[c][j] = a[piv][j]; a[piv][j] = tmp; }
            sign = -sign;
        }
        const double d = a[c][c];
        if (d < 0) sign = -sign;
        logabs += log(fabs(d));
        const double inv = 1.0 / d;
        for (int j = 0; j < 2 * n; ++j) a[c][j] *= inv;
        for (int r = 0; r < n; ++r) {
            if (r == c) continue;
            const double f = a[r][c];
            if (f == 0.0) continue;
            for (int j = 0; j < 2 * n; ++j) a[r][j] -= f * a[c][j];
        }
    }
    if (logdet_out) *logdet_out = sign > 0 ? (float)(logabs * (double)scale) : __builtin_nanf("");
    if (inv_out)
        for (int i = 0; i < n; ++i)
            for (int j = 0; j < n; ++j) inv_out[i * n + j] = (float)a[i][n + j];
}
static __device__ __forceinline__ void small_logdet_one(const SmallMatJob& j, float scale, double (*a)[32]) {
    const int n = (int)j.n;
    for (int i = 0; i < n; ++i)
        for (int c = 0; c < n; ++c) {
            a[i][c] = j.W[i * n + c];
            a[i][n + c] = (i == c) ? 1.0 : 0.0;
        }
    double logabs = 0.0;
    int sign = 1;
    for (int c = 0; c < n; ++c) {
        int piv = c;
        double best = fabs(a[c][c]);
        for (int r = c + 1; r < n; ++r)
            if (fabs(a[r][c]) > best) { best = fabs(a[r][c]); piv = r; }
        if (piv != c) {
            for (int q = 0; q < 2 * n; ++q) { double tmp = a[c][q]; a[c][q] = a[piv][q]; a[piv][q] = tmp; }
            sign = -sign;
        }
        const double d = a[c][c];
        if (d < 0) sign = -sign;
        logabs += log(fabs(d));
        const double inv = 1.0 / d;
        for (int q = 0; q < 2 * n; ++q) a[c][q] *= inv;
        for (int r = 0; r < n; ++r) {
            if (r == c) continue;
            const double f = a[r][c];
            if (f == 0.0) continue;
            for (int q = 0; q < 2 * n; ++q) a[r][q] -= f * a[c][q];
        }
    }
    if (j.logdet_out) *j.logdet_out = sign > 0 ? (float)(logabs * (double)scale) : __builtin_nanf("");
    if (j.inv_out)
        for (int i = 0; i < n; ++i)
            for (int c = 0; c < n; ++c) j.inv_out[i * n + c] = (float)a[i][n + c];
}
__global__ void small_logdet_batch_kernel(const SmallMatJob* jobs, float scale) {
    __shared__ double a[16][32];
    if (threadIdx.x != 0) return;
    small_logdet_one(jobs[blockIdx.x], scale, a);
}
struct SmallMatJobs16 { SmallMatJob j[16]; };
__global__ void small_logdet_batch_val_kernel(const SmallMatJobs16 jobs, float scale) {
    __shared__ double a[16][32];
    if (threadIdx.x != 0) return;
    small_logdet_one(jobs.j[blockIdx.x], scale, a);
}
hipError_t t2s_launch_small_logdet_batch(const SmallMatJob* jobs, int n_jobs, float scale, hipStream_t stream) {
    hipLaunchKernelGGL(small_logdet_batch_kernel, dim3(n_jobs), dim3(64), 0, stream, jobs, scale);
    return hipGetLastError();
}
hipError_t t2s_launch_small_logdet_batch_host(const SmallMatJob* host_jobs, int n_jobs, float scale, hipStream_t stream) {
    if (n_jobs > 16) return hipErrorInvalidValue;
    SmallMatJobs16 v;
    memset(&v, 0, sizeof(v));
    for (int i = 0; i < n_jobs; ++i) v.j[i] = host_jobs[i];
    hipLaunchKernelGGL(small_logdet_batch_val_kernel, dim3(n_jobs), dim3(64), 0, stream, v, scale);
    return hipGetLastError();
}

hipError_t t2s_launch_small_logdet_inv(const float* W, int n, float scale, float* logdet_out, float* inv_out,
                                       hipStream_t stream) {
    hipLaunchKernelGGL(small_logdet_inv_kernel, dim3(1), dim3(64), 0, stream, W, n, scale, logdet_out, inv_out);
    return hipGetLastError();
}

#define START_TT 8
static __device__ __forceinline__ void start_fold_term(float x, int set, bool is_weight, u16& hi, u16& lo) {
    u16 h, l;
    split_bf16(x, h, l);
    hi = h;
    lo = l;
    if (set == (is_weight ? 1 : 2)) {
        split_bf16(x - join_bf16(h, l), hi, lo);
    } else if (set == 3) {
        hi = l;
        lo = 0;
    }
}
template <bool RAG, class FMT = T2sFmt>
__global__ __launch_bounds__(256) void start_kernel(const float* __restrict__ z, const float* __restrict__ w,
                                                    const float* __restrict__ bias, int G, int c_off, int nh, int C,
                                                    int L, int Lp, int halo, u16* X_hi, u16* X_lo, int taps, int nwc,
                                                    u16* W_hi, u16* W_lo, const int* __restrict__ lengths) {
    const int tid = threadIdx.x;
    const int q = tid & 3;
    const int tbase = blockIdx.x * (64 * START_TT) + (tid >> 2);
    const int chunk = blockIdx.y;
    const int b = blockIdx.z;
    const int c8 = chunk * 32 + q * 8;
    int lim = L;
    if constexpr (RAG) lim = min(max(lengths[b], 0), L);
    float wv[8][8], bv[8];
#pragma unroll
    for (int e = 0; e < 8; ++e) {
        const int c = c8 + e;
        bv[e] = c < C ? bias[c] : 0.f;
#pragma unroll
        for (int j = 0; j < 8; ++j) wv[e][j] = (c < C && j < nh) ? w[c * nh + j] : 0.f;
    }
    const int nchunks = (C + 31) / 32;
    const size_t row0 = ((size_t)b * nchunks + chunk) * Lp + halo;
#pragma unroll 2
    for (int it = 0; it < START_TT; ++it) {
        const int t = tbase + it * 64;
        if (t >= L) break;
        if constexpr (RAG) {
            if (t >= lim) {
                *(uint4*)(X_hi + (row0 + t) * 32 + q * 8) = make_uint4(0, 0, 0, 0);
                *(uint4*)(X_lo + (row0 + t) * 32 + q * 8) = make_uint4(0, 0, 0, 0);
                continue;
            }
        }
        float a0[8];
#pragma unroll
        for (int j = 0; j < 8; ++j) a0[j] = j < nh ? z[((size_t)b * G + c_off + j) * L + t] : 0.f;
        u16 hi[8], lo[8];
#pragma unroll
        for (int e = 0; e < 8; ++e) {
            float v = bv[e];
#pragma unroll
            for (int j = 0; j < 8; ++j)
                if (j < nh) v += wv[e][j] * a0[j];
            split_fmt<FMT>(v, hi[e], lo[e]);
        }
        uint4 ph, pl;
        ph.x = hi[0] | ((uint32_t)hi[1] << 16); ph.y = hi[2] | ((uint32_t)hi[3] << 16);
        ph.z = hi[4] | ((uint32_t)hi[5] << 16); ph.w = hi[6] | ((uint32_t)hi[7] << 16);
        pl.x = lo[0] | ((uint32_t)lo[1] << 16); pl.y = lo[2] | ((uint32_t)lo[3] << 16);
        pl.z = lo[4] | ((uint32_t)lo[5] << 16); pl.w = lo[6] | ((uint32_t)lo[7] << 16);
        *(uint4*)(X_hi + (row0 + t) * 32 + q * 8) = ph;
        *(uint4*)(X_lo + (row0 + t) * 32 + q * 8) = pl;
    }
    if (W_hi == nullptr || chunk >= nwc) return;
    const int nw = nh + 1, ncol = taps * nw, spc = 4 / nwc;
    const size_t wrow0 = ((size_t)b * nwc + chunk) * Lp + halo;
    for (int it = 0; it < START_TT; ++it) {
        const int t = tbase + it * 64;
        if (t >= L) break;
        u16 hi[8], lo[8];
#pragma unroll
        for (int e = 0; e < 8; ++e) {
            const int col = q * 8 + e;
            const int sidx = col / ncol, c = col - sidx * ncol;
            const int tap = c / nw, j = c - tap * nw;
            const int tt = t + tap - (taps >> 1);
            float v = 0.f;
            if (sidx < spc && tt >= 0 && tt < lim) v = j < nh ? z[((size_t)b * G + c_off + j) * L + tt] : 1.0f;
            start_fold_term(v, chunk * spc + sidx, false, hi[e], lo[e]);
        }
        uint4 ph, pl;
        ph.x = hi[0] | ((uint32_t)hi[1] << 16); ph.y = hi[2] | ((uint32_t)hi[3] << 16);
        ph.z = hi[4] | ((uint32_t)hi[5] << 16); ph.w = hi[6] | ((uint32_t)hi[7] << 16);
        pl.x = lo[0] | ((uint32_t)lo[1] << 16); pl.y = lo[2] | ((uint32_t)lo[3] << 16);
        pl.z = lo[4] | ((uint32_t)lo[5] << 16); pl.w = lo[6] | ((uint32_t)lo[7] << 16);
        *(uint4*)(W_hi + (wrow0 + t) * 32 + q * 8) = ph;
        *(uint4*)(W_lo + (wrow0 + t) * 32 + q * 8) = pl;
    }
}
hipError_t t2s_launch_start(const float* z, const float* w, const float* bias, int B, int n_group, int c_off,
                            int n_half, int C, int L, int Lp, int halo, u16* X_hi, u16* X_lo, hipStream_t stream,
                            int taps, int nwc, u16* W_hi, u16* W_lo, const int* lengths, bool h16) {
    dim3 grid((L + 64 * START_TT - 1) / (64 * START_TT), (C + 31) / 32, B);
    if (h16) {
        if (W_hi || W_lo) return hipErrorInvalidValue;
        if (lengths)
            hipLaunchKernelGGL((start_kernel<true, T2sFmtF16>), grid, dim3(256), 0, stream, z, w, bias, n_group, c_off, n_half, C, L,
                               Lp, halo, X_hi, X_lo, 0, 0, (u16*)nullptr, (u16*)nullptr, lengths);
        else
            hipLaunchKernelGGL((start_kernel<false, T2sFmtF16>), grid, dim3(256), 0, stream, z, w, bias, n_group, c_off, n_half, C, L,
                               Lp, halo, X_hi, X_lo, 0, 0, (u16*)nullptr, (u16*)nullptr, (const int*)nullptr);
        return hipGetLastError();
    }
    if (lengths)
        hipLaunchKernelGGL(start_kernel<true>, grid, dim3(256), 0, stream, z, w, bias, n_group, c_off, n_half, C, L, Lp, halo,
                           X_hi, X_lo, taps, nwc, W_hi, W_lo, lengths);
    else
        hipLaunchKernelGGL(start_kernel<false>, grid, dim3(256), 0, stream, z, w, bias, n_group, c_off, n_half, C, L, Lp, halo,
                           X_hi, X_lo, taps, nwc, W_hi, W_lo, lengths);
    return hipGetLastError();
}

__global__ __launch_bounds__(256) void end_affine_kernel(const float* __restrict__ skip, const float* __restrict__ w_end,
                                                         const float* __restrict__ b_end, float* z, float* log_s,
                                                         float* wn_out, int G, int c_off, int nh, int C, int L, int Lp,
                                                         int halo, int reverse) {
    const int tid = threadIdx.x;
    const int l32 = tid & 31;
    const int t = blockIdx.x * 8 + (tid >> 5);
    const int b = blockIdx.y;
    const int nj = 2 * nh;
    const int nchunks = (C + 31) / 32;
    float part[16];
#pragma unroll
    for (int j = 0; j < 16; ++j) part[j] = 0.f;
    const bool tv = t < L;
    if (tv) {
        for (int ck = 0; ck < nchunks; ++ck) {
            const int c = ck * 32 + l32;
// ... 16 lines not shown
        float bb = 0.f, ls = 0.f;
#pragma unroll
        for (int j = 0; j < 16; ++j) {
            if (j == l32) bb = part[j];
            if (j == nh + l32) ls = part[j];
        }
        bb += b_end[l32];
        ls += b_end[nh + l32];
        float* zp = z + ((size_t)b * G + c_off + nh + l32) * L + t;
        const float a1 = *zp;
        *zp = reverse ? (a1 - bb) / expf(ls) : expf(ls) * a1 + bb;
        if (log_s) log_s[((size_t)b * nh + l32) * L + t] = ls;
        if (wn_out) {
            wn_out[((size_t)b * 2 * nh + l32) * L + t] = bb;
            wn_out[((size_t)b * 2 * nh + nh + l32) * L + t] = ls;
        }
    }
}
hipError_t t2s_launch_end_affine(const float* skip, const float* w_end, const float* b_end, float* z, float* log_s,
                                 float* wn_out, int B, int n_group, int c_off, int n_half, int C, int L, int Lp, int halo,
                                 int reverse, hipStream_t stream) {
    hipLaunchKernelGGL(end_affine_kernel, dim3((L + 7) / 8, B), dim3(256), 0, stream, skip, w_end, b_end, z, log_s, wn_out,
                       n_group, c_off, n_half, C, L, Lp, halo, reverse);
    return hipGetLastError();
}

#define EF_OROWS 8
#define EF_PART (8 * 33)
typedef const float __attribute__((address_space(1))) * ef_gptr;
typedef float ef_f4 __attribute__((ext_vector_type(4)));
template <bool VEC>
static __device__ __forceinline__ float4 endfold_load4(ef_gptr v, int o, int c0, int C) {
    ef_gptr p = v + (size_t)min(o, C - 1) * C;
    if (VEC) {
        const ef_f4 t = *(const ef_f4 __attribute__((address_space(1))) *)(p + min(c0, C - 4));
        return make_float4(t.x, t.y, t.z, t.w);
    }
    return make_float4(p[min(c0, C - 1)], p[min(c0 + 1, C - 1)], p[min(c0 + 2, C - 1)], p[min(c0 + 3, C - 1)]);
}
template <bool VEC>
static __device__ __forceinline__ void endfold_block(const EndFoldJob& j, int C, int Cp, float* s_ef, float* s_bes) {
    const int tid = threadIdx.x, s = tid >> 3, cq = tid & 7;
    const int nj = (int)j.nj;
    const int c0 = blockIdx.y * 32 + cq * 4;
    ef_gptr v = (ef_gptr)j.v_skip;
    float4 x[EF_OROWS], xn[EF_OROWS];
#pragma unroll
    for (int e = 0; e < EF_OROWS; ++e) x[e] = endfold_load4<VEC>(v, s + 32 * e, c0, C);
    ef_gptr w_end = (ef_gptr)j.w_end, scale = (ef_gptr)j.scale, b_skip = (ef_gptr)j.b_skip;
    const bool with_bes = blockIdx.y == 0;
    float bsum[8];
#pragma unroll
    for (int r = 0; r < 8; ++r) bsum[r] = 0.f;
    for (int ob = 0; ob < Cp; ob += 512) {
        float sc[2], bk[2], wv[2][8];
#pragma unroll
        for (int u = 0; u < 2; ++u) {
            const int o = ob + u * 256 + tid;
            const bool ok = o < C;
            sc[u] = (ok && scale) ? scale[o] : 1.f;
            bk[u] = (ok && with_bes) ? b_skip[o] : 0.f;
#pragma unroll
            for (int r = 0; r < 8; ++r) wv[u][r] = (ok && r < nj) ? w_end[(size_t)r * C + o] : 0.f;
        }
#pragma unroll
        for (int u = 0; u < 2; ++u) {
            const int o = ob + u * 256 + tid;
            if (o < Cp) {
#pragma unroll
                for (int r = 0; r < 8; ++r) {
                    s_ef[r * Cp + o] = wv[u][r] * sc[u];
                    bsum[r] += wv[u][r] * bk[u];
                }
            }
        }
    }
    if (with_bes) {
#pragma unroll
        for (int r = 0; r < 8; ++r) {
            const float t = wave_sum(bsum[r]);
            if ((tid & 63) == 0) s_bes[(tid >> 6) * 8 + r] = t;
        }
    }
    __syncthreads();
    if (with_bes && tid < 8) j.bes[tid] = s_bes[tid] + s_bes[8 + tid] + s_bes[16 + tid] + s_bes[24 + tid];
    float acc[8][4];
#pragma unroll
    for (int r = 0; r < 8; ++r) acc[r][0] = acc[r][1] = acc[r][2] = acc[r][3] = 0.f;
    for (int o0 = 0; o0 < C; o0 += 32 * EF_OROWS) {
        const int o1 = o0 + 32 * EF_OROWS;
        if (o1 < C) {
#pragma unroll
            for (int e = 0; e < EF_OROWS; ++e) xn[e] = endfold_load4<VEC>(v, o1 + s + 32 * e, c0, C);
        }
#pragma unroll
        for (int e = 0; e < EF_OROWS; ++e) {
            const float* w = s_ef + o0 + s + 32 * e;
#pragma unroll
            for (int r = 0; r < 8; ++r) {
                acc[r][0] += w[r * Cp] * x[e].x;
                acc[r][1] += w[r * Cp] * x[e].y;
                acc[r][2] += w[r * Cp] * x[e].z;
                acc[r][3] += w[r * Cp] * x[e].w;
            }
        }
#pragma unroll
        for (int e = 0; e < EF_OROWS; ++e) x[e] = xn[e];
    }
    __syncthreads();
#pragma unroll
    for (int r = 0; r < 8; ++r) {
        float* p = s_ef + s * EF_PART + r * 33 + cq * 4;
        p[0] = acc[r][0]; p[1] = acc[r][1]; p[2] = acc[r][2]; p[3] = acc[r][3];
    }
    __syncthreads();
}
template <class FMT = T2sFmt>
__global__ __launch_bounds__(256) void endfold_weights_kernel(const EndFoldJob* __restrict__ jobs, int C) {
    extern __shared__ float s_ef[];
    __shared__ float s_bes[4 * 8];
    const EndFoldJob j = jobs[blockIdx.x];
    const int tid = threadIdx.x;
    const int Cp = (C + 32 * EF_OROWS - 1) & ~(32 * EF_OROWS - 1);
    if (!(C & 3) && !((uintptr_t)j.v_skip & 15)) endfold_block<true>(j, C, Cp, s_ef, s_bes);
    else endfold_block<false>(j, C, Cp, s_ef, s_bes);
    {
        const int q = tid >> 6, r = (tid >> 3) & 7, e = tid & 7;
        const int cl = (e >> 2) * 16 + q * 4 + (e & 3);
        float sum = 0.f;
#pragma unroll 8
        for (int sl = 0; sl < 32; ++sl) sum += s_ef[sl * EF_PART + r * 33 + cl];
        if (blockIdx.y * 32 + cl < C) {
            u16* base = j.fold_A + (size_t)blockIdx.y * 2 * 64 * 8;
            u16 h, l;
            split_fmt<FMT>(sum, h, l);
            const int lane = q * 16 + r;
            base[(size_t)lane * 8 + e] = h;
            base[(size_t)(64 + lane) * 8 + e] = l;
        }
    }
}
hipError_t t2s_launch_endfold_weights(const EndFoldJob* jobs, int n_jobs, int C, hipStream_t stream, bool h16) {
    const int Cp = (C + 32 * EF_OROWS - 1) & ~(32 * EF_OROWS - 1);
    const int lds_floats = 8 * Cp > 32 * EF_PART ? 8 * Cp : 32 * EF_PART;
    if (h16)
        hipLaunchKernelGGL((endfold_weights_kernel<T2sFmtF16>), dim3(n_jobs, (C + 31) / 32), dim3(256),
                           (size_t)lds_floats * sizeof(float), stream, jobs, C);
    else
    hipLaunchKernelGGL((endfold_weights_kernel<>), dim3(n_jobs, (C + 31) / 32), dim3(256), (size_t)lds_floats * sizeof(float),
                       stream, jobs, C);
    return hipGetLastError();
}

__global__ __launch_bounds__(256) void startfold_weights_kernel(const float* __restrict__ v, const float* __restrict__ g,
                                                                const float* __restrict__ w_start,
                                                                const float* __restrict__ b_start, int C, int nh, int Kt,
                                                                int Mpad, int nwc, u16* A_hi, u16* A_lo) {
    extern __shared__ float s_sf[];
    const int tid = threadIdx.x, wave = tid >> 6, lane = tid & 63, nwaves = blockDim.x >> 6;
    const int nw = nh + 1, n = C * Kt, O = 2 * C;
    float* xs = s_sf + ((C * nw + 3) & ~3) + (size_t)wave * ((n + 3) & ~3);
    const int o = blockIdx.x * nwaves + wave;
    const bool row_ok = o < O;
    const float* vrow = v + (size_t)(row_ok ? o : 0) * n;
    float ss = 0.f;
    const bool vec = !(n & 3) && !((uintptr_t)v & 15);
    const int bd = blockDim.x, nws = C * nh;
    if (!vec) {
        for (int i = lane; i < n; i += 64) {
            const float x = vrow[i];
            xs[i] = x;
            ss += x * x;
        }
    }
    for (int b = 0;; ++b) {
        const int v0 = b * 2048 + lane * 4, w0 = b * 8 * bd + tid, b0 = b * 2 * bd + tid;
        if ((!vec || b * 2048 >= n) && b * 8 * bd >= nws && b * 2 * bd >= C) break;
        float4 xr[8];
        float wr[8], br[2];
#pragma unroll
        for (int k = 0; k < 8; ++k)
            xr[k] = (vec && v0 + k * 256 < n) ? *(const float4*)(vrow + v0 + k * 256) : make_float4(0.f, 0.f, 0.f, 0.f);
#pragma unroll
        for (int k = 0; k < 8; ++k) wr[k] = w0 + k * bd < nws ? w_start[w0 + k * bd] : 0.f;
#pragma unroll
        for (int k = 0; k < 2; ++k) br[k] = b0 + k * bd < C ? b_start[b0 + k * bd] : 0.f;
#pragma unroll
        for (int k = 0; k < 8; ++k) {
            if (vec && v0 + k * 256 < n) {
                *(float4*)(xs + v0 + k * 256) = xr[k];
                ss += xr[k].x * xr[k].x + xr[k].y * xr[k].y + xr[k].z * xr[k].z + xr[k].w * xr[k].w;
            }
        }
#pragma unroll
        for (int k = 0; k < 8; ++k) {
            const int i = w0 + k * bd;
            if (i < nws) {
                const int c = i / nh;
                s_sf[c * nw + (i - c * nh)] = wr[k];
            }
        }
#pragma unroll
        for (int k = 0; k < 2; ++k)
            if (b0 + k * bd < C) s_sf[(b0 + k * bd) * nw + nh] = br[k];
    }
    ss = wave_sum(ss);
    const float scale = g ? g[row_ok ? o : 0] / sqrtf(ss) : 1.0f;
    __syncthreads();
    if (!row_ok) return;
    const int half = lane >> 5, col = lane & 31;
    const int ncol = Kt * nw, spc = 4 / nwc;
    const int sidx = col / ncol, lc = col - sidx * ncol;
    float acc = 0.f;
    if (sidx < spc) {
        const int tap = lc / nw, j = lc - tap * nw;
        const int ch = (C + 1) >> 1, c1 = half ? C : ch;
#pragma unroll 8
        for (int c = half ? ch : 0; c < c1; ++c) acc += xs[c * Kt + tap] * s_sf[c * nw + j];
    }
    acc += __shfl_xor(acc, 32, 64);
    const int gate = o >= C;
    const int ch = gate ? o - C : o;
    const int p = (ch >> 7) * 256 + ((ch >> 6) & 1) * 128 + (((ch >> 4) & 3) * 2 + gate) * 16 + (ch & 15);
    u16* A = half ? A_lo : A_hi;
    for (int wc = 0; wc < nwc; ++wc) {
        u16 h, l;
        start_fold_term(acc * scale, wc * spc + sidx, true, h, l);
        A[((size_t)wc * Mpad + p) * 32 + col] = half ? l : h;
    }
}
hipError_t t2s_launch_startfold_weights(const float* v, const float* g, const float* w_start, const float* b_start, int C,
                                        int n_half, int taps, int Mpad, int nwc, u16* A_hi, u16* A_lo, hipStream_t stream) {
    const size_t wb = (size_t)((C * (n_half + 1) + 3) & ~3), row = (size_t)((C * taps + 3) & ~3);
    int rows = 4;
    while (rows > 1 && (wb + rows * row) * sizeof(float) > 65536) rows >>= 1;
    hipLaunchKernelGGL(startfold_weights_kernel, dim3((2 * C + rows - 1) / rows), dim3(64 * rows),
                       (wb + rows * row) * sizeof(float), stream, v, g, w_start, b_start, C, n_half, taps, Mpad, nwc, A_hi, A_lo);
    return hipGetLastError();
}

__global__ void end_fold_affine_kernel(const float* __restrict__ fold_acc, int nslots, const float* __restrict__ bes,
                                       int n_layers, const float* __restrict__ b_end, float* z, float* log_s, float* wn_out,
                                       int B, int G, int c_off, int nh, int L, int reverse) {
    const int t = blockIdx.x * blockDim.x + threadIdx.x;
    const int i = blockIdx.y, b = blockIdx.z;
    if (t >= L) return;
    float bb = b_end[i], ls = b_end[nh + i];
    for (int l = 0; l < n_layers; ++l) { bb += bes[l * 8 + i]; ls += bes[l * 8 + nh + i]; }
    for (int s = 0; s < nslots; ++s) {
        bb += fold_acc[(((size_t)s * B + b) * 8 + i) * L + t];
        ls += fold_acc[(((size_t)s * B + b) * 8 + nh + i) * L + t];
    }
    float* zp = z + ((size_t)b * G + c_off + nh + i) * L + t;
    const float a1 = *zp;
    *zp = reverse ? (a1 - bb) / expf(ls) : expf(ls) * a1 + bb;
    if (log_s) log_s[((size_t)b * nh + i) * L + t] = ls;
    if (wn_out) {
        wn_out[((size_t)b * 2 * nh + i) * L + t] = bb;
        wn_out[((size_t)b * 2 * nh + nh + i) * L + t] = ls;
    }
}
hipError_t t2s_launch_end_fold_affine(const float* fold_acc, int nslots, const float* bes, int n_layers,
                                      const float* b_end, float* z, float* log_s, float* wn_out, int B, int n_group, int c_off,
                                      int n_half, int L, int reverse, hipStream_t stream) {
    hipLaunchKernelGGL(end_fold_affine_kernel, dim3((L + 255) / 256, n_half, B), dim3(256), 0, stream, fold_acc, nslots, bes,
                       n_layers, b_end, z, log_s, wn_out, B, n_group, c_off, n_half, L, reverse);
    return hipGetLastError();
}

#define FB_TC 64
#define FB_EDGE 32
template <bool RAG>
__global__ __launch_bounds__(256) void flow_boundary_kernel(const FlowBoundaryArgs a) {
    __shared__ float zs[16][FB_TC + FB_EDGE];
    __shared__ float zo[16][FB_TC + FB_EDGE];
    __shared__ float ws[16 * 16];
    const int tid = threadIdx.x, b = blockIdx.y;
    const int G = a.G, L = a.L;
    const int hw = a.taps >> 1, tce = FB_TC + 2 * hw;
    const int t0 = blockIdx.x * FB_TC, te0 = t0 - hw;
    if (a.W && tid < a.n_rem * a.n_rem) ws[tid] = a.W[tid];
    for (int idx = tid; idx < G * tce; idx += 256) {
        const int g = idx / tce, lc = idx - g * tce, t = te0 + lc;
        zs[g][lc] = (t >= 0 && t < L) ? a.z_in[((size_t)b * G + g) * L + t] : 0.f;
    }
    __syncthreads();
    if (a.fold_acc) {
        const int nh = a.nh_prev, B = gridDim.y;
        for (int idx = tid; idx < nh * tce; idx += 256) {
            const int i = idx / tce, lc = idx - i * tce, t = te0 + lc;
            if (t < 0 || t >= L) continue;
            float bb = a.b_end[i], ls = a.b_end[nh + i];
            for (int l = 0; l < a.n_layers; ++l) { bb += a.bes[l * 8 + i]; ls += a.bes[l * 8 + nh + i]; }
            for (int s = 0; s < a.nslots; ++s) {
                bb += a.fold_acc[(((size_t)s * B + b) * 8 + i) * L + t];
                ls += a.fold_acc[(((size_t)s * B + b) * 8 + nh + i) * L + t];
            }
            const int g = a.c_off_prev + nh + i;
            const float a1 = zs[g][lc];
            zs[g][lc] = expf(ls) * a1 + bb;
            if (a.log_s && lc >= hw && lc < hw + FB_TC) a.log_s[((size_t)b * nh + i) * L + t] = ls;
        }
        __syncthreads();
    }
    if (a.W) {
        const int n = a.n_rem;
        for (int idx = tid; idx < n * tce; idx += 256) {
            const int i = idx / tce, lc = idx - i * tce;
            float s = 0.f;
            for (int j = 0; j < n; ++j) s += ws[i * n + j] * zs[a.c_off + j][lc];
            zo[i][lc] = s;
        }
        __syncthreads();
    }
    const int c_lo = a.W ? a.c_off : G, c_hi = a.W ? a.c_off + a.n_rem : G;
    auto col = [&](int g, int lc) { return (g >= c_lo && g < c_hi) ? zo[g - c_lo][lc] : zs[g][lc]; };
    if (a.z_out) {
        for (int idx = tid; idx < G * FB_TC; idx += 256) {
            const int g = idx / FB_TC, r = idx - g * FB_TC, t = t0 + r;
            if (t < L) a.z_out[((size_t)b * G + g) * L + t] = col(g, r + hw);
        }
    }
    const int nh = a.nh, nw = nh + 1, ncol = a.taps * nw, nwc = a.nwc, spc = 4 / nwc;
    int lim = L;
    if constexpr (RAG) lim = min(max(a.lengths[b], 0), L);
    for (int idx = tid; idx < FB_TC * nwc * 4; idx += 256) {
        const int q = idx & 3, rc = idx >> 2, chunk = rc % nwc, r = rc / nwc, t = t0 + r;
        if (t >= L) continue;
        u16 hi[8], lo[8];
#pragma unroll
        for (int e = 0; e < 8; ++e) {
            const int cc = q * 8 + e;
            const int sidx = cc / ncol, c = cc - sidx * ncol;
            const int tap = c / nw, j = c - tap * nw;
            const int tt = t + tap - hw;
            float v = 0.f;
            if (sidx < spc && tt >= 0 && tt < lim) v = j < nh ? col(a.c_off + j, r + tap) : 1.0f;
            start_fold_term(v, chunk * spc + sidx, false, hi[e], lo[e]);
        }
        uint4 ph, pl;
        ph.x = hi[0] | ((uint32_t)hi[1] << 16); ph.y = hi[2] | ((uint32_t)hi[3] << 16);
        ph.z = hi[4] | ((uint32_t)hi[5] << 16); ph.w = hi[6] | ((uint32_t)hi[7] << 16);
        pl.x = lo[0] | ((uint32_t)lo[1] << 16); pl.y = lo[2] | ((uint32_t)lo[3] << 16);
        pl.z = lo[4] | ((uint32_t)lo[5] << 16); pl.w = lo[6] | ((uint32_t)lo[7] << 16);
        const size_t o = (((size_t)b * nwc + chunk) * a.Lp + a.halo + t) * 32 + q * 8;
        *(uint4*)(a.W_hi + o) = ph;
        *(uint4*)(a.W_lo + o) = pl;
    }
}
int t2s_flow_boundary_max_taps() { return FB_EDGE + 1; }
hipError_t t2s_launch_flow_boundary(const FlowBoundaryArgs& a, int B, hipStream_t stream) {
    const dim3 grid((a.L + FB_TC - 1) / FB_TC, B);
    if (a.lengths) hipLaunchKernelGGL(flow_boundary_kernel<true>, grid, dim3(256), 0, stream, a);
    else hipLaunchKernelGGL(flow_boundary_kernel<false>, grid, dim3(256), 0, stream, a);
    return hipGetLastError();
}
```

text2speech_amd/glow.py:

```python
import ctypes
import os
from collections import namedtuple

import torch
import torch.nn.functional as F

from . import _lib


class _WaveGlowLossFn(torch.autograd.Function):

    @staticmethod
    def forward(ctx, sigma, n_flows, z, *rest):
        log_s = [t.detach().to(torch.float32).contiguous() for t in rest[:n_flows]]
        dets = [t.detach() for t in rest[n_flows:]]
        d0 = dets[0]
        if all(t.dtype == torch.float32 and t.dim() == 0 and t.untyped_storage().data_ptr() == d0.untyped_storage().data_ptr()
               and t.storage_offset() == d0.storage_offset() + k for k, t in enumerate(dets)):
            log_det = d0.as_strided((n_flows,), (1,))
        else:
            log_det = torch.stack([t.to(torch.float32).reshape(()) for t in dets])
        zc = z.detach().to(torch.float32).contiguous()
        dev = zc.device
        d_z = torch.empty_like(zc) if z.requires_grad else None
# ... 74 lines not shown

    def __init__(self, n_in_channels, n_mel_channels, n_layers, n_channels, kernel_size):
        super().__init__()
        assert kernel_size % 2 == 1
        assert n_channels % 2 == 0
        self.n_layers = n_layers
        self.n_channels = n_channels
        self.kernel_size = kernel_size
        self.in_layers = torch.nn.ModuleList()
        self.res_skip_layers = torch.nn.ModuleList()
        self.cond_layers = torch.nn.ModuleList()
        wn = torch.nn.utils.weight_norm
        self.start = wn(torch.nn.Conv1d(n_in_channels, n_channels, 1), name="weight")
        end = torch.nn.Conv1d(n_channels, 2 * n_in_channels, 1)
        end.weight.data.zero_()
        end.bias.data.zero_()
        self.end = end
        for i in range(n_layers):
            dilation = 2 ** i
            padding = (kernel_size * dilation - dilation) // 2
            self.in_layers.append(wn(torch.nn.Conv1d(n_channels, 2 * n_channels, kernel_size,
                                                     dilation=dilation, padding=padding), name="weight"))
            self.cond_layers.append(wn(torch.nn.Conv1d(n_mel_channels, 2 * n_channels, 1), name="weight"))
            rs = 2 * n_channels if i < n_layers - 1 else n_channels
            self.res_skip_layers.append(wn(torch.nn.Conv1d(n_channels, rs, 1), name="weight"))

    def __getstate__(self):
        d = self.__dict__.copy()
        d.pop("_owner", None)
        return d

    def forward(self, forward_input):
        ref = self.__dict__.get("_owner")
        owner = ref() if ref is not None else None
        if owner is None:
            raise _lib.T2SError("WN.forward runs on the engine of the WaveGlow it belongs to; build it through WaveGlow(...)")
        audio, spect = forward_input
        with torch.no_grad():
            return owner._eng().wn_forward(self.__dict__["_flow"], audio, spect)


def _vg(conv):
    if hasattr(conv, "weight_v"):
        return conv.weight_v, conv.weight_g
    return conv.weight, None


def _f32c(t):
    return t.detach().to(torch.float32).contiguous()


_Path = namedtuple("_Path", "start_fold boundary compose")

_Plan = namedtuple("_Plan", "path h16 lens entry pk melwin")

_ENTRY_POINTS = {
    "pack":         ("t2s_pack_conv_weight_table", "t2s_pack_conv_weight_table",
                     "t2s_pack_conv_weight_table_h16", "t2s_pack_conv_weight_table_h16"),
    "endfold":      ("t2s_wg_endfold_weights", "t2s_wg_endfold_weights", "t2s_wg_endfold_weights_h16", "t2s_wg_endfold_weights_h16"),
    "upsample":     ("t2s_wg_upsample_squeeze", "t2s_wg_upsample_squeeze", "t2s_wg_upsample_squeeze_h16", "t2s_wg_upsample_squeeze_h16"),
    "boundary":     ("t2s_wg_flow_boundary", "t2s_wg_flow_boundary_ragged", None, None),
    "start":        ("t2s_wg_start", "t2s_wg_start_ragged", "t2s_wg_start_h16", "t2s_wg_start_h16_ragged"),
    "start_window": ("t2s_wg_start_window", "t2s_wg_start_ragged", None, None),
    "gate":         ("t2s_wg_in_cond_gate_fold", "t2s_wg_in_cond_gate_fold",
                     "t2s_wg_in_cond_gate_fold_h16", "t2s_wg_in_cond_gate_fold_h16_ragged"),
    "gate_window":  ("t2s_wg_in_win_gate_fold", "t2s_wg_in_win_gate_fold", None, None),
    "gate_melwin":  ("t2s_wg_in_melwin_gate_fold", None, None, None),
    "res":          ("t2s_wg_res_only", "t2s_wg_res_only_ragged", "t2s_wg_res_only_h16", "t2s_wg_res_only_h16_ragged"),
    "res_start":    ("t2s_wg_res_only_start", "t2s_wg_res_only_start_ragged", None, None),
}
_TAKES_LENGTHS = {
    "t2s_wg_flow_boundary_ragged": "t2s_wg_flow_boundary",
    "t2s_wg_start_ragged": "t2s_wg_start_window",
    "t2s_wg_res_only_ragged": "t2s_wg_res_only",
    "t2s_wg_res_only_start_ragged": "t2s_wg_res_only_start",
    "t2s_wg_start_h16_ragged": "t2s_wg_start_h16",
    "t2s_wg_in_cond_gate_fold_h16_ragged": "t2s_wg_in_cond_gate_fold_h16",
    "t2s_wg_res_only_h16_ragged": "t2s_wg_res_only_h16",
}
_START_TAKES_WINDOW = ("t2s_wg_start_window", "t2s_wg_start_ragged")


def _entry_point(stage, h16, ragged=False):
    return _ENTRY_POINTS[stage][2 * bool(h16) + bool(ragged)]

_INFER_W16_AUTO = True


class _Engine:

    def __init__(self, model):
        self.m = model
        self.packed = None
        self.packed_key = None
        self.ws = {}
        self.last_path = None
        self.infer_w16 = None
        self.last_infer_w16 = False
        self.infer_batch_w16 = False
        self.last_infer_batch_w16 = False
        self.packed16 = None
        self.packed16_key = None
        self._keep = []
        self._streams = {}
        self.grad_sync = None
        self.gemm_events = None
        self.gemm_event_stride = 1
        self._gemm_launch_no = 0

    def geom(self):
        m = self.m
        wn0 = m.WN[0]
        C, nl, ks = wn0.n_channels, wn0.n_layers, wn0.kernel_size
        n_cond = m.upsample.out_channels * m.n_group
        halo = -(-((2 ** (nl - 1)) * (ks // 2)) // 32) * 32
        g = dict(C=C, nl=nl, ks=ks, n_cond=n_cond, Cpad=-(-C // 32) * 32, Spad=-(-n_cond // 32) * 32,
                 halo=halo, Mpad1=-(-C // 128) * 256)
        g["ncol0"] = ks * (m.n_group // 2 + 1)
        g["nwc"] = 2 if 2 * g["ncol0"] <= 32 else 4
        g["nk1"] = ks * g["Cpad"] // 32 + g["Spad"] // 32
        g["nk2"] = g["Cpad"] // 32
        return g

    def path(self, compose=True):
        g = self.geom()
        if g["C"] % 16:
            raise _lib.T2SError("WaveGlow's forward without gradients, infer and WN.forward need n_channels %% 16 == 0, not %d" % g["C"])
        compose = self.compose_geom() if compose else None
        start_fold = (compose is None and os.environ.get("T2S_START_FOLD", "1") != "0" and g["ncol0"] <= 32
                      and g["Cpad"] // 32 >= g["nwc"])
        boundary = (start_fold and os.environ.get("T2S_FLOW_BOUNDARY", "1") != "0" and g["C"] % 32 == 0 and g["nl"] >= 2
                    and self.m.n_group // 2 <= 4)
        return _Path(start_fold, boundary, compose)

    def train_check(self):
        g = self.geom()
        if g["C"] % 32:
            raise _lib.T2SError("WaveGlow's forward with gradients (training) needs n_channels %% 32 == 0, not %d" % g["C"])

    def start_fold_on(self):
        return self.path().start_fold

    def _plan(self, h16=False, lens=None):
        path = self.last_path = _Path(False, False, None) if h16 else self.path(compose=lens is None)
        lengths = () if lens is None else (_lib.ptr(lens),)
        entry = {}
        for stage in _ENTRY_POINTS:
            name = _entry_point(stage, h16, lens is not None)
            entry[stage] = (name, lengths if name in _TAKES_LENGTHS else ())
        return _Plan(path, h16, lens, entry, None, None)

    def _pack(self, plan, device, force=False, flow_events=None):
        return plan._replace(pk=self.pack_weights(device, force=force, flow_events=flow_events, res_pair8=True,
                                                  start_fold=plan.path.start_fold, h16=plan.h16))

    def _stream(self, name, device):
        key = (name, str(device))
        if key not in self._streams:
            self._streams[key] = torch.cuda.Stream(device=device)
        return self._streams[key]

    def pack_weights(self, device, force=True, flow_events=None, res_pair8=False, start_fold=False, h16=False):
        assert not (h16 and (start_fold or flow_events is not None))
        res_pair8 = bool(res_pair8) and self.geom()["C"] % 32 == 0
        key = tuple(p._version for p in self.m.parameters()) + (str(device), res_pair8, start_fold)
        slot = "packed16" if h16 else "packed"
        pk = getattr(self, slot)
        if (h16 or not force) and pk is not None and getattr(self, slot + "_key") == key:
            return pk
        if pk is None or pk["device"] != device:
            pk = dict(flows=self._alloc_planes(device, h16), device=device, h16=h16)
            setattr(self, slot, pk)
        srcs = self._pack_jobs(pk, res_pair8, start_fold)
        fsrcs = self._fold_jobs(pk)
        starts = self._launch_pack(pk, start_fold, flow_events)
        setattr(self, slot + "_key", key)
        pk["res_pair8"] = res_pair8
        pk["start_fold"] = start_fold
        pk["keep"] = srcs + fsrcs + starts
        return pk

    def w16_eligible(self, batch=False):
        if batch:
            return False, "infer_batch stays on split-bf16 planes"
        if any(p.dtype != torch.float16 for wn in self.m.WN for p in wn.parameters()):
            return False, "not every WN parameter is torch.float16 (a .half() model)"
        if self.geom()["C"] % 16:
            return False, "n_channels %% 16 != 0 (%d)" % self.geom()["C"]
        if _lib.operand_format() != 0:
            return False, "the loaded library is the fp16-operand diagnostic build"
        return True, ""

    def use_w16(self, batch=False):
        if self.infer_w16 is False:
            return False
        ok, why = self.w16_eligible(batch)
        if self.infer_w16 is True and not ok:
            raise _lib.T2SError("infer_w16 = True: %s" % why)
        return ok and (self.infer_w16 is True or _INFER_W16_AUTO)

    _W16_BATCH_SYMBOLS = ("t2s_wg_start_h16_ragged", "t2s_wg_in_cond_gate_fold_h16_ragged", "t2s_wg_res_only_h16_ragged")

    def w16_batch_eligible(self):
        ok, why = self.w16_eligible(batch=False)
        if not ok:
            return False, why
        lib = _lib.load()
        missing = [n for n in self._W16_BATCH_SYMBOLS if not hasattr(lib, n)]
        if missing:
            return False, "the loaded library does not export %s" % ", ".join(missing)
        return True, ""

    def use_batch_w16(self):
        if self.infer_batch_w16 is not True:
            return False
        ok, why = self.w16_batch_eligible()
        if not ok:
            raise _lib.T2SError("infer_batch_w16 = True: %s" % why)
        return True

    def _alloc_planes(self, device, h16=False):
        m, g = self.m, self.geom()
        C, nl = g["C"], g["nl"]
        f32 = dict(dtype=torch.float32, device=device)
        plane = lambda *shape: torch.zeros(*shape, dtype=torch.float16 if h16 else torch.bfloat16, device=device)
        bf16_only = (lambda *shape: None) if h16 else plane
        a0 = (g["nwc"] + g["Spad"] // 32, g["Mpad1"], 32)
        flows = []
        for k in range(m.n_flows):
            n_half = m.WN[k].start.in_channels
            layers = []
            for i in range(nl):
                rows2 = 2 * C if i < nl - 1 else C
                Mpad2 = _lib.padded_rows(rows2)
                layers.append(dict(
                    A1h=plane(g["nk1"], g["Mpad1"], 32), A1l=bf16_only(g["nk1"], g["Mpad1"], 32), b1=torch.zeros(g["Mpad1"], **f32),
                    A2h=plane(g["nk2"], Mpad2, 32), A2l=bf16_only(g["nk2"], Mpad2, 32), b2=torch.zeros(Mpad2, **f32), Mpad2=Mpad2,
                    s_in=torch.empty(2 * C, **f32), s_cond=torch.empty(2 * C, **f32), s_rs=torch.empty(rows2, **f32),
                    fold_A=plane(-(-C // 128) * 8192)))
            flows.append(dict(layers=layers, n_half=n_half, bes=torch.zeros(nl, 8, **f32), w_start=torch.empty(C, n_half, **f32),
                              A0h=bf16_only(*a0), A0l=bf16_only(*a0), w_inv=None))
        return flows

    def _pack_jobs(self, pk, res_pair8, start_fold):
        m, g = self.m, self.geom()
        C, nl, ks = g["C"], g["nl"], g["ks"]
        srcs = []
        specs = []
        for k, wn in enumerate(m.WN):
            fl = pk["flows"][k]
            specs.append([])
            for i in range(nl):
                ly = fl["layers"][i]
                v, gg = _vg(wn.in_layers[i])
                vc, gc = _vg(wn.cond_layers[i])
                vr, gr = _vg(wn.res_skip_layers[i])
                t = [_f32c(v), None if gg is None else _f32c(gg), _f32c(wn.in_layers[i].bias), _f32c(wn.cond_layers[i].bias),
                     _f32c(vc), None if gc is None else _f32c(gc),
                     _f32c(vr), None if gr is None else _f32c(gr), _f32c(wn.res_skip_layers[i].bias)]
                srcs += t
                if i == 0 and start_fold:
                    specs[k].append((t[4], t[5], t[2], t[3], fl["A0h"], fl["A0l"], ly["b1"], 2 * C, g["n_cond"], 1, 1, C,
                                     g["Mpad1"], 32 * g["nwc"], g["Spad"], ly["s_cond"]))
                else:
                    specs[k].append((t[0], t[1], t[2], t[3], ly["A1h"], ly["A1l"], ly["b1"], 2 * C, C, ks, 1, C, g["Mpad1"], 0,
                                     g["Cpad"], ly["s_in"]))
                    specs[k].append((t[4], t[5], None, None, ly["A1h"], ly["A1l"], None, 2 * C, g["n_cond"], 1, 1, C, g["Mpad1"],
                                     ks * g["Cpad"], g["Spad"], ly["s_cond"]))
                p8 = res_pair8 and i < nl - 1
                specs[k].append((t[6], t[7], t[8], None, ly["A2h"], ly["A2l"], ly["b2"], t[6].size(0), C, 1, 2 if p8 else 0,
                                 C if p8 else 0, ly["Mpad2"], 0, g["Cpad"], ly["s_rs"]))
        ptr_key = tuple(0 if t is None else t.data_ptr() for t in srcs) + (res_pair8, start_fold)
        if pk.get("job_key") != ptr_key:
            rows, flow_rows, flow_jobs = [], [], []
            dp = lambda t: 0 if t is None else t.data_ptr()
            for fspecs in specs:
                row_start = 0
                flow_jobs.append((len(rows), len(fspecs)))
                for (v, gg, b1, b2, Ah, Al, bo, O, Cin, Kt, perm, Cg, Mpad, koff, Cin_pad, so) in fspecs:
                    rows.append([dp(v), dp(gg), dp(b1), dp(b2), dp(Ah), dp(Al), dp(bo), row_start,
                                 O, Cin, Kt, perm, Cg, Mpad, koff, Cin_pad, 0, 0, dp(so)])
                    row_start += -(-O // 16)
                flow_rows.append(row_start)
            pk["jobs"] = torch.tensor(rows, dtype=torch.int64).to(pk["device"])
            pk["flow_rows"] = flow_rows
            pk["flow_jobs"] = flow_jobs
            pk["job_key"] = ptr_key
        return srcs

    def _fold_jobs(self, pk):
        m, g = self.m, self.geom()
        C, nl = g["C"], g["nl"]
        fsrc = []
        for k, wn in enumerate(m.WN):
            fl = pk["flows"][k]
            w_end = _f32c(wn.end.weight)
            for i in range(nl):
                vr = _f32c(_vg(wn.res_skip_layers[i])[0])
                br = _f32c(wn.res_skip_layers[i].bias)
                r0 = C if i < nl - 1 else 0
                fsrc.append((w_end, vr, br, r0, fl["layers"][i], fl["bes"], i, 2 * fl["n_half"]))
        fkey = tuple((a.data_ptr(), b.data_ptr(), c.data_ptr()) for a, b, c, *_ in fsrc)
        if pk.get("fold_key") != fkey:
            rows = []
            for (w_end, vr, br, r0, ly, bes, i, nj) in fsrc:
                rows.append([w_end.data_ptr(), vr.data_ptr() + 4 * r0 * C, ly["s_rs"].data_ptr() + 4 * r0,
                             br.data_ptr() + 4 * r0, ly["fold_A"].data_ptr(), bes.data_ptr() + 4 * 8 * i, nj, C])
            pk["fold_jobs"] = torch.tensor(rows, dtype=torch.int64).to(pk["device"])
            pk["fold_key"] = fkey
        return [t for tup in fsrc for t in tup[:3]]

    def _launch_pack(self, pk, start_fold, flow_events):
        m, g = self.m, self.geom()
        C, nl, ks = g["C"], g["nl"], g["ks"]
        st = _lib.current_stream()
        jobs_ptr, fold_ptr = pk["jobs"].data_ptr(), pk["fold_jobs"].data_ptr()
        pack, endfold = _entry_point("pack", pk["h16"]), _entry_point("endfold", pk["h16"])
        starts = []
        for k, wn in enumerate(m.WN):
            fl = pk["flows"][k]
            j0, nj = pk["flow_jobs"][k]
            _lib.call(pack, _lib.c_vp(jobs_ptr + j0 * 19 * 8), nj, pk["flow_rows"][k], st)
            _lib.call(endfold, _lib.c_vp(fold_ptr + k * nl * 8 * 8), nl, C, st)
            v, gg = _vg(wn.start)
            v, gg = _f32c(v), (None if gg is None else _f32c(gg))
            starts += [v, gg]
            _lib.call("t2s_weightnorm_small", _lib.ptr(v), _lib.ptr(gg), C, fl["n_half"], _lib.ptr(fl["w_start"]), st)
            if start_fold:
                v0, g0 = _vg(wn.in_layers[0])
                v0, g0, b_start = _f32c(v0), (None if g0 is None else _f32c(g0)), _f32c(wn.start.bias)
                starts += [v0, g0, b_start]
                _lib.call("t2s_wg_startfold_weights", _lib.ptr(v0), _lib.ptr(g0), _lib.ptr(fl["w_start"]),
                          _lib.ptr(b_start), C, fl["n_half"], ks, g["Mpad1"], g["nwc"], _lib.ptr(fl["A0h"]), _lib.ptr(fl["A0l"]), st)
            fl["w_inv"] = None
            if flow_events is not None:
                ev = torch.cuda.Event()
                ev.record()
                flow_events.append(ev)
        return starts

    def compose_geom(self):
        m, g = self.m, self.geom()
        up = m.upsample
        ksz, stride, G = up.kernel_size[0], up.stride[0], m.n_group
        if os.environ.get("T2S_COND_COMPOSE") != "1":
            return None
        if ksz % stride or stride % G or ((ksz // stride) * up.in_channels) % 32 or g["C"] % 16:
            return None
        return stride // G, ksz // stride, (ksz // stride) * up.in_channels

    def compose_cond(self, device):
        if self.packed.get("compose_key") == self.packed_key:
            return
        m, g = self.m, self.geom()
        P, nlag, K2 = self.compose_geom()
        C, nl, ks = g["C"], g["nl"], g["ks"]
        up = m.upsample
        st = _lib.current_stream()
        ncols = P * K2 + 1
        Lp_u = _lib.plane_rows(ncols, 0)
        sc = g["Spad"] // 32
        bf = dict(dtype=torch.bfloat16, device=device)
        U_h, U_l = torch.zeros(1, sc, Lp_u, 32, **bf), torch.zeros(1, sc, Lp_u, 32, **bf)
        W, bias = _f32c(up.weight), _f32c(up.bias)
        _lib.call("t2s_wg_upsample_basis", _lib.ptr(W), _lib.ptr(bias), up.in_channels, up.kernel_size[0], up.stride[0],
                  m.n_group, Lp_u, 0, _lib.ptr(U_h), _lib.ptr(U_l), st)
        tmp = torch.empty(2 * C, ncols, dtype=torch.float32, device=device)
        zb = torch.zeros(g["Mpad1"], dtype=torch.float32, device=device)
        cond_off = (ks * g["Cpad"] // 32) * g["Mpad1"] * 32 * 2
        mc = K2 // 32
        for k in range(m.n_flows):
            for i in range(nl):
                ly = self.packed["flows"][k]["layers"][i]
                if "Ach" not in ly:
                    ly["Ach"] = torch.zeros(P, mc, g["Mpad1"], 32, **bf)
                    ly["Acl"] = torch.zeros(P, mc, g["Mpad1"], 32, **bf)
                    ly["b1c"] = torch.zeros(g["Mpad1"], dtype=torch.float32, device=device)
                _lib.call("t2s_conv_bias_act", _lib.c_vp(ly["A1h"].data_ptr() + cond_off), _lib.c_vp(ly["A1l"].data_ptr() + cond_off),
                          _lib.ptr(zb), _lib.ptr(U_h), _lib.ptr(U_l), None, None, _lib.ptr(tmp), 0, 1, g["n_cond"], 2 * C, 1, 1, 0,
                          ncols, Lp_u, 0, g["Mpad1"], st)
                _lib.call("t2s_wg_compose_cond", _lib.ptr(tmp), _lib.ptr(ly["b1"]), 2 * C, g["Mpad1"], P, K2, ncols,
                          _lib.ptr(ly["Ach"]), _lib.ptr(ly["Acl"]), _lib.ptr(ly["b1c"]), st)
        self._keep += [U_h, U_l, tmp, zb, W, bias]
        self.packed["compose_key"] = self.packed_key

    def workspace(self, B, L, device):
        key = (B, L, str(device))
        w = self.ws.get(key)
        if w is None:
            g = self.geom()
            Lp = _lib.plane_rows(L, g["halo"])
            bf = dict(dtype=torch.bfloat16, device=device)
            xc, sc = g["Cpad"] // 32, g["Spad"] // 32
            w = dict(Lp=Lp,
                     Xh=torch.zeros(B, xc, Lp, 32, **bf), Xl=torch.zeros(B, xc, Lp, 32, **bf),
                     Ah=torch.zeros(B, xc, Lp, 32, **bf), Al=torch.zeros(B, xc, Lp, 32, **bf),
                     Sh=torch.zeros(B, sc, Lp, 32, **bf), Sl=torch.zeros(B, sc, Lp, 32, **bf),
                     Wh=torch.zeros(B, g["nwc"], Lp, 32, **bf), Wl=torch.zeros(B, g["nwc"], Lp, 32, **bf),
                     z2=torch.empty(B, self.m.n_group, L, dtype=torch.float32, device=device),
                     fold_acc=torch.zeros(_lib.load().t2s_wg_gate_fold_slots(B, g["C"], L), B, 8, L, dtype=torch.float32,
                                          device=device))
            self.ws = {key: w}
        return w

    def _check_inputs(self, *tensors):
        for t in tensors:
            if not t.is_cuda:
                raise _lib.T2SError("WaveGlow (MI355X build) needs CUDA/HIP tensors; got a %s tensor - there is no "
                                    "CPU fallback" % t.device)

    def _upsample(self, mel, B, L, w, plan=None):
        m, g = self.m, self.geom()
        up = m.upsample
        mel32 = _f32c(mel)
        W, bias = _f32c(up.weight), _f32c(up.bias)
        name = plan.entry["upsample"][0] if plan is not None else _entry_point("upsample", False)
        _lib.call(name, _lib.ptr(mel32), _lib.ptr(W), _lib.ptr(bias), B, up.in_channels,
                  mel32.size(2), up.kernel_size[0], up.stride[0], m.n_group, L, w["Lp"], g["halo"],
                  _lib.ptr(w["Sh"]), _lib.ptr(w["Sl"]), _lib.current_stream())
        self._keep += [mel32, W, bias]

    def _boundary(self, plan, k, z_in, z_out, B, L, w, prev=None, W=None):
        m, g = self.m, self.geom()
        c_off, n_rem, n_half = self._flow_geom(k)
        fold_acc = bes = b_end = log_s = None
        nslots = c_off_p = nh_p = 0
        if prev is not None:
            kp, log_s = prev
            c_off_p, _, nh_p = self._flow_geom(kp)
            fold_acc, nslots = w["fold_acc"], w["fold_acc"].size(0)
            bes = plan.pk["flows"][kp]["bes"]
            b_end = _f32c(m.WN[kp].end.bias)
            self._keep.append(b_end)
        name, lengths = plan.entry["boundary"]
        _lib.call(name, _lib.ptr(z_in), _lib.ptr(z_out), _lib.ptr(fold_acc), nslots, _lib.ptr(bes), g["nl"],
                  _lib.ptr(b_end), _lib.ptr(log_s), c_off_p, nh_p, _lib.ptr(W), c_off, n_rem, n_half, B, m.n_group, L, w["Lp"],
                  g["halo"], g["ks"], g["nwc"], _lib.ptr(w["Wh"]), _lib.ptr(w["Wl"]), *lengths, _lib.current_stream())

    def _wn(self, plan, k, z, B, L, w, c_off, n_half):
        m, g = self.m, self.geom()
        C, nl, ks = g["C"], g["nl"], g["ks"]
        path, P = plan.path, _lib.ptr
        fl = plan.pk["flows"][k]
        st = _lib.current_stream()
        b_start = _f32c(m.WN[k].start.bias)
        self._keep.append(b_start)
        X, S, win, acts = ((P(w[n + "h"]), P(w[n + "l"])) for n in "XSWA")
        if not path.boundary:
            name, lengths = plan.entry["start_window" if path.start_fold else "start"]
            window = ()
            if name in _START_TAKES_WINDOW:
                window = (ks, g["nwc"], *win) if path.start_fold else (0, 0, None, None)
            _lib.call(name, P(z), P(fl["w_start"]), P(b_start), B, m.n_group, c_off, n_half, C, L, w["Lp"], g["halo"], *X,
                      *window, *lengths, st)
        gate, gate_lengths = plan.entry["gate" if plan.melwin is None else "gate_melwin"]
        gate_window = plan.entry["gate_window"][0]
        res, res_lengths = plan.entry["res"]
        res_start, res_start_lengths = plan.entry["res_start"]
        pair8 = 1 if plan.pk["res_pair8"] else 0
        dims1 = (L, w["Lp"], g["halo"], g["Mpad1"])
        for i in range(nl):
            ly = fl["layers"][i]
            full_k = not (path.start_fold and i == 0)
            timed = full_k and self.gemm_events is not None and self._gemm_launch_no % self.gemm_event_stride == 0
            if full_k:
                self._gemm_launch_no += 1
            if timed:
                e0, e1 = torch.cuda.Event(enable_timing=True), torch.cuda.Event(enable_timing=True)
                e0.record()
            out = (*acts, P(ly["fold_A"]), P(w["fold_acc"]))
            if not full_k:
                _lib.call(gate_window, P(fl["A0h"]), P(fl["A0l"]), P(ly["b1"]), *win, *S, *out, 1, B, C, g["n_cond"], g["nwc"], *dims1, st)
            elif plan.melwin is not None:
                Mh, Ml, Fp, n_phase, K2 = plan.melwin
                _lib.call(gate, P(ly["A1h"]), P(ly["A1l"]), P(ly["Ach"]), P(ly["Acl"]), P(ly["b1c"]), *X, P(Mh), P(Ml), *out,
                          1 if i == 0 else 0, B, C, K2, ks, 2 ** i, *dims1, n_phase, Fp, st)
            else:
                _lib.call(gate, P(ly["A1h"]), P(ly["A1l"]), P(ly["b1"]), *X, *S, *out,
                          1 if i == 0 else 0, B, C, g["n_cond"], ks, 2 ** i, *dims1, *gate_lengths, st)
            if timed:
                e1.record()
                self.gemm_events.append((e0, e1))
            if i == nl - 1:
                continue
            weights = (P(ly["A2h"]), P(ly["A2l"]), P(ly["b2"]), *acts)
            dims2 = (B, C, L, w["Lp"], g["halo"], ly["Mpad2"])
            if path.boundary and i == 0:
                _lib.call(res_start, *weights, P(z), P(fl["w_start"]), P(b_start), m.n_group, c_off, n_half, *X, *dims2,
                          *res_start_lengths, st)
            else:
                _lib.call(res, *weights, *X, *dims2, pair8, *res_lengths, st)

    def wn_forward(self, k, audio, spect):
        self._check_inputs(audio, spect)
        dev = audio.device
        B, n_in, L = audio.shape
        c_off, n_rem, n_half = self._flow_geom(k)
        g = self.geom()
        if n_in != n_half or spect.size(1) != g["n_cond"] or spect.size(2) != L:
            raise ValueError("WN[%d] takes audio [B, %d, L] and spect [B, %d, L]" % (k, n_half, g["n_cond"]))
        plan = self._plan()
        self._keep = []
        plan = self._pack(plan, dev)
        w = self.workspace(B, L, dev)
        st = _lib.current_stream()
        spect32 = _f32c(spect)
        _lib.call("t2s_f32_to_planes", _lib.ptr(spect32), B, g["n_cond"], L, w["Lp"], g["halo"], _lib.ptr(w["Sh"]), _lib.ptr(w["Sl"]), st)
        z = torch.zeros(B, self.m.n_group, L, dtype=torch.float32, device=dev)
        z[:, c_off:c_off + n_half] = audio.detach().to(torch.float32)
        if plan.path.boundary:
            self._boundary(plan, k, z, None, B, L, w)
        self._wn(plan, k, z, B, L, w, c_off, n_half)
        wn_out =torch.empty(B, 2 * n_half, L, dtype=torch.float32, device=dev)
        self._end_fold(k, z, None, w["fold_acc"], wn_out, B, L, c_off, n_half, reverse=False, plan=plan)
        self._keep += [spect32, z]
        return wn_out.to(audio.dtype)

    def _end_fold(self, k, z, log_s, fold_acc, wn_out, B, L, c_off, n_half, reverse, plan=None):
        b_end = _f32c(self.m.WN[k].end.bias)
        self._keep.append(b_end)
        pk = self.packed if plan is None else plan.pk
        _lib.call("t2s_wg_end_fold_affine", _lib.ptr(fold_acc), fold_acc.size(0), _lib.ptr(pk["flows"][k]["bes"]),
                  self.geom()["nl"], _lib.ptr(b_end), _lib.ptr(z), _lib.ptr(log_s), _lib.ptr(wn_out), B, self.m.n_group, c_off,
                  n_half, L, 1 if reverse else 0, _lib.current_stream())

    def _end_skip(self, k, z, log_s, skip, wn_out, Lp, B, L, c_off, n_half):
        g, wn = self.geom(), self.m.WN[k]
        w_end, b_end = _f32c(wn.end.weight), _f32c(wn.end.bias)
        self._keep += [w_end, b_end]
        _lib.call("t2s_wg_end_affine", _lib.ptr(skip), _lib.ptr(w_end), _lib.ptr(b_end), _lib.ptr(z), _lib.ptr(log_s),
                  _lib.ptr(wn_out), B, self.m.n_group, c_off, n_half, g["C"], L, Lp, g["halo"], 0, _lib.current_stream())

    def _flow_geom(self, k):
        m = self.m
        c_off = m.n_early_size * (k // m.n_early_every)
        n_rem = m.n_group - c_off
        return c_off, n_rem, n_rem // 2

    def logdet_jobs(self, Ws, log_det, inverses=None):
        return torch.tensor([[Ws[k].data_ptr(), log_det.data_ptr() + 4 * k, 0 if inverses is None else inverses[k].data_ptr(),
                              self._flow_geom(k)[1]] for k in range(self.m.n_flows)], dtype=torch.int64)

    def forward(self, mel, audio):
        m = self.m
        self._check_inputs(mel, audio)
        dev = audio.device
        B, T = audio.shape
        G = m.n_group
        L = T // G
        up = m.upsample
        if (mel.size(2) - 1) * up.stride[0] + up.kernel_size[0] < T:
            raise AssertionError("upsampled spectrogram shorter than audio (reference glow.py:216)")
        plan = self._plan()
        path = plan.path
        self._keep = []
        w = self.workspace(B, L, dev)
        main = torch.cuda.current_stream(dev)
        side = self._stream("side", dev)
        audio32 = _f32c(audio)
        z = torch.empty(B, G, L, dtype=torch.float32, device=dev)
        if path.boundary:
            bufs = [z, w["z2"]] if m.n_flows % 2 == 0 else [w["z2"], z]
            z = bufs[0]
        log_s_list, log_det_list = [], []
        log_det = torch.empty(m.n_flows, dtype=torch.float32, device=dev)
        Ws = [_f32c(m.convinv[k].conv.weight) for k in range(m.n_flows)]
        use_val = m.n_flows <= 16
        jobs = self.logdet_jobs(Ws, log_det)
        if not use_val:
            jobs = jobs.to(dev)
        self._keep += [audio32, jobs] + Ws
        side.wait_stream(main)
        with torch.cuda.stream(side):
            st2 = _lib.current_stream()
            _lib.call("t2s_wg_audio_squeeze", _lib.ptr(audio32), _lib.ptr(z), B, T, G, L, 0, st2)
            self._upsample(mel, B, L, w, plan)
            ev_inputs = torch.cuda.Event()
            ev_inputs.record()
            if use_val:
                _lib.call("t2s_small_logdet_inv_batch_host", ctypes.c_void_p(jobs.data_ptr()), m.n_flows, float(B * L), st2)
            else:
                _lib.call("t2s_small_logdet_inv_batch", _lib.ptr(jobs), m.n_flows, float(B * L), st2)
        pack_s = self._stream("pack", dev)
        pack_events = []
        pack_s.wait_stream(main)
        with torch.cuda.stream(pack_s):
            plan = self._pack(plan, dev, force=True, flow_events=pack_events)
        main.wait_event(ev_inputs)
        st = _lib.current_stream()
        for k in range(m.n_flows):
            main.wait_event(pack_events[k])
            c_off, n_rem, n_half = self._flow_geom(k)
            log_s = torch.empty(B, n_half, L, dtype=torch.float32, device=dev)
            if path.boundary:
                z_out = bufs[(k + 1) % 2]
                self._boundary(plan, k, z, z_out, B, L, w, prev=(k - 1, log_s_list[k - 1]) if k else None, W=Ws[k])
                z = z_out
            else:
                _lib.call("t2s_wg_convinv", _lib.ptr(z), _lib.ptr(Ws[k]), B, G, c_off, n_rem, L, st)
            self._wn(plan, k, z, B, L, w, c_off, n_half)
            if not path.boundary or k == m.n_flows - 1:
                self._end_fold(k, z, log_s, w["fold_acc"], None, B, L, c_off, n_half, reverse=False, plan=plan)
            log_s_list.append(log_s)
            log_det_list.append(log_det[k])
        main.wait_stream(side)
        return z, log_s_list, log_det_list

    def infer(self, mel, sigma, noise):
        return self._infer(mel, sigma, noise, None)

    def infer_batch(self, mel, lengths, sigma, noise):
        m = self.m
        self._check_inputs(mel)
        stride = m.upsample.stride[0]
        lens = (lengths * (stride // m.n_group)).to(torch.int32).to(mel.device)
        audio = self._infer(mel, sigma, noise, lens)
        B, T = audio.shape
        _lib.call("t2s_zero_rows_f32", _lib.ptr(audio), _lib.ptr(lens), B, T // m.n_group, m.n_group, _lib.current_stream())
        self._keep.append(lens)
        return audio, (lengths * stride).to(mel.device)

    def _infer(self, mel, sigma, noise, lens):
        m = self.m
        self._check_inputs(mel)
        dev = mel.device
        B, _, frames = mel.shape
        G = m.n_group
        up = m.upsample
        T = (frames - 1) * up.stride[0] + up.kernel_size[0] - (up.kernel_size[0] - up.stride[0])
        L = T // G
        batch = lens is not None
        batch_w16 = self.last_infer_batch_w16 = batch and self.use_batch_w16()
        h16 = self.last_infer_w16 = batch_w16 or self.use_w16(batch=batch)
        plan = self._plan(h16, lens)
        path = plan.path
        self._keep = []
        plan = self._pack(plan, dev)
        w = self.workspace(B, L, dev)
        st = _lib.current_stream()
        if path.compose is not None and _lib.load().t2s_wg_gate_tile_rows(B, self.geom()["C"], L) == 256:
            P, nlag, K2 = path.compose
            self.compose_cond(dev)
            Fp = -(-frames // 256) * 256
            key = ("melwin", B, Fp, str(dev))
            mw = self.ws.get(key)
            if mw is None:
                mw = (torch.zeros(B, K2 // 32, Fp, 32, dtype=torch.bfloat16, device=dev),
                      torch.zeros(B, K2 // 32, Fp, 32, dtype=torch.bfloat16, device=dev))
                self.ws[key] = mw
            mel32 = _f32c(mel)
            _lib.call("t2s_wg_melwin_planes", _lib.ptr(mel32), B, mel32.size(1), frames, nlag, Fp, _lib.ptr(mw[0]), _lib.ptr(mw[1]), st)
            self._keep.append(mel32)
            plan = plan._replace(melwin=(mw[0], mw[1], Fp, P, K2))
        else:
            self._upsample(mel, B, L, w, plan)
        z = torch.empty(B, G, L, dtype=torch.float32, device=dev)
        n_rem_final = m.n_remaining_channels
        early_ks = [k for k in reversed(range(m.n_flows)) if k % m.n_early_every == 0 and k > 0]
        if noise is None:
            noise_final = torch.randn(B, n_rem_final, L, dtype=torch.float32, device=dev)
            noise_early = [torch.randn(B, m.n_early_size, L, dtype=torch.float32, device=dev) for _ in early_ks]
        else:
            noise_final, noise_early = noise
        z[:, G - n_rem_final:] = sigma * noise_final.to(dev, torch.float32)
        for k, ne in zip(early_ks, noise_early):
            c_off = m.n_early_size * (k // m.n_early_every)
            z[:, c_off - m.n_early_size:c_off] = sigma * ne.to(dev, torch.float32)
        for k in reversed(range(m.n_flows)):
            c_off, n_rem, n_half = self._flow_geom(k)
            fl = plan.pk["flows"][k]
            if fl["w_inv"] is None:
                Wk = _f32c(m.convinv[k].conv.weight)
                fl["w_inv"] = torch.empty(n_rem, n_rem, dtype=torch.float32, device=dev)
                _lib.call("t2s_small_logdet_inv", _lib.ptr(Wk), n_rem, 1.0, None, _lib.ptr(fl["w_inv"]), st)
                fl["_Wk"] = Wk
            if path.boundary:
                self._boundary(plan, k, z, None, B, L, w)
            self._wn(plan, k, z, B, L, w, c_off, n_half)
            self._end_fold(k, z, None, w["fold_acc"], None, B, L, c_off, n_half, reverse=True, plan=plan)
            _lib.call("t2s_wg_convinv", _lib.ptr(z), _lib.ptr(fl["w_inv"]), B, G, c_off, n_rem, L, st)
        audio = torch.empty(B, L * G, dtype=torch.float32, device=dev)
        _lib.call("t2s_wg_audio_squeeze", _lib.ptr(audio), _lib.ptr(z), B, L * G, G, L, 1, st)
        return audio


class WaveGlow(torch.nn.Module):

    def __init__(self, n_mel_channels, n_flows, n_group, n_early_every, n_early_size, WN_config):
        super().__init__()
        self.upsample = torch.nn.ConvTranspose1d(n_mel_channels, n_mel_channels, 1024, stride=256)
        assert n_group % 2 == 0
        self.n_flows = n_flows
        self.n_group = n_group
        self.n_early_every = n_early_every
        self.n_early_size = n_early_size
        self.WN = torch.nn.ModuleList()
        self.convinv = torch.nn.ModuleList()
        n_half = n_group // 2
        n_remaining_channels = n_group
        for k in range(n_flows):
            if k % self.n_early_every == 0 and k > 0:
                n_half = n_half - self.n_early_size // 2
                n_remaining_channels = n_remaining_channels - self.n_early_size
            self.convinv.append(Invertible1x1Conv(n_remaining_channels))
            self.WN.append(WN(n_half, n_mel_channels * n_group, **WN_config))
        self.n_remaining_channels = n_remaining_channels
        self.__dict__["_engine"] = None
        self._adopt()

    def _adopt(self):
        import weakref
        for k, wn_k in enumerate(self.WN):
            wn_k.__dict__["_owner"] = weakref.ref(self)
            wn_k.__dict__["_flow"] = k

    def __setstate__(self, state):
        super().__setstate__(state)
        if "_engine" not in self.__dict__:
            self.__dict__["_engine"] = None
        self._adopt()

    def _eng(self):
        if self.__dict__.get("_engine") is None:
            self.__dict__["_engine"] = _Engine(self)
        return self.__dict__["_engine"]

    def __getstate__(self):
        d = self.__dict__.copy()
        d["_engine"] = None
        return d

    def forward(self, forward_input):
        spect, audio = forward_input
        f16 = _lib.operand_format() == 1
        if torch.is_grad_enabled() and any(p.requires_grad for p in self.parameters()):
# ... 84 lines not shown
```

Baseline: 8.139 million audio samples/s.

## Batch startfold weights, widen pack kernel, parallelize logdet, split end-fold res packing

Replaces per-flow weightnorm and startfold launches with a table-driven startfold kernel that computes the start weight normalisation inline. The first flow is launched alone and the rest are batched right after it. The pack kernel now spreads each row across four waves and uses 16-byte vectorised loads and stores. The small-matrix logdet/inverse now runs its Gauss-Jordan elimination across a 64-lane wave instead of a single thread. The logdet launch is moved ahead of the audio squeeze on the side stream, and with end_fold the skip rows of the res-skip weights are no longer packed into planes. These changes aim to cut weight-preparation time and launch count, which sit on the critical path of each forward. The cost is added kernel complexity, including inline normalisation that recomputes per-element sums.

Result: no change. 8.174 million audio samples/s, median of 6 (+0.4%).

```diff
diff --git a/include/t2s_hip.h b/include/t2s_hip.h
--- a/include/t2s_hip.h
+++ b/include/t2s_hip.h
@@ -88,6 +88,14 @@
                         void* stream);
 int t2s_wg_startfold_weights(const float* v_in, const float* g_in, const float* w_start, const float* b_start, int C, int n_half,
                              int taps, int Mpad, int win_chunks, void* A_hi, void* A_lo, void* stream);
+typedef struct t2s_startfold_job {
+    const float *v_in, *g_in, *v_start, *g_start, *b_start;
+    float* w_start;
+    void *A_hi, *A_lo;
+    long n_half;
+} t2s_startfold_job;
+int t2s_wg_startfold_weights_table(const t2s_startfold_job* host_jobs, int n_jobs, int C, int taps, int Mpad, int win_chunks,
+                                   void* stream);
 int t2s_wg_in_win_gate_fold(const void* A_hi, const void* A_lo, const float* bias, const void* W_hi, const void* W_lo,
                             const void* S_hi, const void* S_lo, void* acts_hi, void* acts_lo, const void* fold_A,
                             float* fold_acc, int fold_init, int B, int C, int n_cond, int win_chunks, int L, int Lp, int halo,
diff --git a/text2speech_amd/_lib.py b/text2speech_amd/_lib.py
--- a/text2speech_amd/_lib.py
+++ b/text2speech_amd/_lib.py
@@ -35,6 +35,7 @@
     "t2s_wg_in_cond_gate_fold": [c_vp] * 11 + [c_int] * 10 + [c_vp],
     "t2s_wg_start_window": [c_vp, c_vp, c_vp] + [c_int] * 8 + [c_vp, c_vp, c_int, c_int, c_vp, c_vp, c_vp],
     "t2s_wg_startfold_weights": [c_vp] * 4 + [c_int] * 5 + [c_vp, c_vp, c_vp],
+    "t2s_wg_startfold_weights_table": [c_vp, c_int, c_int, c_int, c_int, c_int, c_vp],
     "t2s_wg_in_win_gate_fold": [c_vp] * 11 + [c_int] * 9 + [c_vp],
     "t2s_wg_gate_fold_slots": [c_int, c_int, c_int],
     "t2s_wg_gate_tile_rows": [c_int, c_int, c_int],
diff --git a/text2speech_amd/csrc/t2s_api.hip b/text2speech_amd/csrc/t2s_api.hip
--- a/text2speech_amd/csrc/t2s_api.hip
+++ b/text2speech_amd/csrc/t2s_api.hip
@@ -236,6 +236,21 @@
     if (Mpad % 256 || Mpad < cdiv(C, 128) * 256 || (size_t)C * (n_half + 1) * sizeof(float) > 60 * 1024) return T2S_EINVAL;
     T2S_CHECK_HIP(t2s_launch_startfold_weights(v_in, g_in, w_start, b_start, C, n_half, taps, Mpad, win_chunks, (u16*)A_hi, (u16*)A_lo,
                                                (hipStream_t)stream));
+    return T2S_OK;
+}
+
+int t2s_wg_startfold_weights_table(const t2s_startfold_job* host_jobs, int n_jobs, int C, int taps, int Mpad, int win_chunks,
+                                   void* stream) {
+    static_assert(sizeof(t2s_startfold_job) == sizeof(StartFoldJob), "t2s_startfold_job layout");
+    if (!host_jobs || n_jobs <= 0 || n_jobs > 16 || C <= 0 || Mpad % 256 || Mpad < cdiv(C, 128) * 256) return T2S_EINVAL;
+    for (int i = 0; i < n_jobs; ++i) {
+        const t2s_startfold_job& j = host_jobs[i];
+        if (!j.v_in || !j.v_start || !j.b_start || !j.w_start || !planes_ok(j.A_hi, j.A_lo)) return T2S_EINVAL;
+        if (j.n_half <= 0 || j.n_half > 8 || !win_chunks_ok(taps, (int)j.n_half, win_chunks)) return T2S_EINVAL;
+        if ((size_t)C * (j.n_half + 1) * sizeof(float) > 60 * 1024) return T2S_EINVAL;
+    }
+    T2S_CHECK_HIP(t2s_launch_startfold_weights_table((const StartFoldJob*)host_jobs, n_jobs, C, taps, Mpad, win_chunks,
+                                                     (hipStream_t)stream));
     return T2S_OK;
 }
 
diff --git a/text2speech_amd/csrc/t2s_kernels.h b/text2speech_amd/csrc/t2s_kernels.h
--- a/text2speech_amd/csrc/t2s_kernels.h
+++ b/text2speech_amd/csrc/t2s_kernels.h
@@ -146,6 +146,16 @@
                             bool h16 = false);
 hipError_t t2s_launch_startfold_weights(const float* v, const float* g, const float* w_start, const float* b_start, int C,
                                         int n_half, int taps, int Mpad, int nwc, u16* A_hi, u16* A_lo, hipStream_t stream);
+struct StartFoldJob {
+    const float* v_in; const float* g_in;
+    const float* v_start; const float* g_start;
+    const float* b_start;
+    float* w_start;
+    u16* A_hi; u16* A_lo;
+    long n_half;
+};
+hipError_t t2s_launch_startfold_weights_table(const StartFoldJob* host_jobs, int n_jobs, int C, int taps, int Mpad, int nwc,
+                                              hipStream_t stream);
 struct EndFoldJob {
     const float* w_end;
     const float* v_skip;
diff --git a/text2speech_amd/csrc/waveglow_ops.hip b/text2speech_amd/csrc/waveglow_ops.hip
--- a/text2speech_amd/csrc/waveglow_ops.hip
+++ b/text2speech_amd/csrc/waveglow_ops.hip
@@ -83,43 +83,47 @@
     *(uint32_t*)(j.A_hi + idx) = h0 | ((uint32_t)h1 << 16);
     if constexpr (!ONE) *(uint32_t*)(j.A_lo + idx) = l0 | ((uint32_t)l1 << 16);
 }
-static __device__ __forceinline__ float sum16(float v) {
-    v += __shfl_xor(v, 1, 64); v += __shfl_xor(v, 2, 64); v += __shfl_xor(v, 4, 64); v += __shfl_xor(v, 8, 64);
-    return v;
-}
 #define PACK_MAX_CHUNKS 20
+#define PACK_WAVE_CHUNKS (PACK_MAX_CHUNKS / 4)
 template <int KT, class FMT, bool ONE>
-static __device__ __forceinline__ void pack_rows_regs(const PackJob& j, int o0) {
-    const int tid = threadIdx.x, r = tid >> 4, cp = tid & 15;
+static __device__ __forceinline__ void pack_rows_wide(const PackJob& j, int o0, float (*s_red)[16]) {
+    const int tid = threadIdx.x, wave = tid >> 6, lane = tid & 63, r = lane >> 2, q = lane & 3;
     const int O = (int)j.O, Cin = (int)j.Cin, Cin_pad = (int)j.Cin_pad, koff = (int)j.koff;
     const int o = o0 + r;
     const bool row_ok = o < O;
-    const int n = Cin * KT;
     const int nchunk = (Cin + 31) >> 5;
-    const float* vrow = j.v + (size_t)(row_ok ? o : 0) * n;
-    float x[PACK_MAX_CHUNKS][2 * KT];
-    float ss = 0.f;
-#pragma unroll
-    for (int cc = 0; cc < PACK_MAX_CHUNKS; ++cc) {
-        const int c = cc * 32 + cp * 2;
+    const bool planes = j.A_hi != nullptr, norm = j.g && !j.g_is_scale;
+    const float* vrow = j.v + (size_t)(row_ok ? o : 0) * Cin * KT;
+    float x[PACK_WAVE_CHUNKS][8 * KT];
+#pragma unroll
+    for (int i = 0; i < PACK_WAVE_CHUNKS; ++i) {
+        const int c0 = (wave + 4 * i) * 32 + q * 8;
+        const bool ok = row_ok && c0 < Cin && (planes || norm);
 #pragma unroll
         for (int e = 0; e < 2 * KT; ++e) {
-            const int ce = c + e / KT;
-            x[cc][e] = (cc < nchunk && row_ok && ce < Cin) ? vrow[c * KT + e] : 0.f;
-            ss += x[cc][e] * x[cc][e];
+            const f32x4 t = ok ? *(const f32x4*)(vrow + c0 * KT + 4 * e) : f32x4{0.f, 0.f, 0.f, 0.f};
+            x[i][4 * e] = t.x; x[i][4 * e + 1] = t.y; x[i][4 * e + 2] = t.z; x[i][4 * e + 3] = t.w;
         }
     }
     float scale = 1.0f;
-    if (j.g) {
-        if (j.g_is_scale) scale = row_ok ? j.g[o] : 1.f;
-        else {
-            ss = sum16(ss);
-            scale = row_ok ? j.g[o] / sqrtf(ss) : 1.f;
-        }
+    if (norm) {
+        float ss = 0.f;
+#pragma unroll
+        for (int i = 0; i < PACK_WAVE_CHUNKS; ++i)
+#pragma unroll
+            for (int e = 0; e < 8 * KT; ++e) ss += x[i][e] * x[i][e];
+        ss += __shfl_xor(ss, 1, 64);
+        ss += __shfl_xor(ss, 2, 64);
+        if (q == 0) s_red[wave][r] = ss;
+        __syncthreads();
+        ss = ((s_red[0][r] + s_red[1][r]) + s_red[2][r]) + s_red[3][r];
+        scale = row_ok ? j.g[o] / sqrtf(ss) : 1.f;
+    } else if (j.g) {
+        scale = row_ok ? j.g[o] : 1.f;
     }
     if (!row_ok) return;
     const int p = pack_dst_row(j, o);
-    if (cp == 0) {
+    if (wave == 0 && q == 0) {
         if (j.scale_out) j.scale_out[o] = scale;
         if (j.bias_out) {
             float bi = j.bias_in ? j.bias_in[o] : 0.f;
@@ -127,13 +131,27 @@
             j.bias_out[p] = bi;
         }
     }
-#pragma unroll
-    for (int cc = 0; cc < PACK_MAX_CHUNKS; ++cc) {
+    if (!planes) return;
+#pragma unroll
+    for (int i = 0; i < PACK_WAVE_CHUNKS; ++i) {
+        const int cc = wave + 4 * i;
         if (cc < nchunk) {
-            const int c = cc * 32 + cp * 2;
-#pragma unroll
-            for (int tap = 0; tap < KT; ++tap)
-                pack_store2<FMT, ONE>(j, koff + tap * Cin_pad + c, p, x[cc][tap] * scale, x[cc][KT + tap] * scale);
+#pragma unroll
+            for (int tap = 0; tap < KT; ++tap) {
+                const int k = koff + tap * Cin_pad + cc * 32 + q * 8;
+                const size_t idx = ((size_t)(k >> 5) * (int)j.Mpad + p) * 32 + (k & 31);
+                uint32_t h[4], l[4];
+#pragma unroll
+                for (int e = 0; e < 4; ++e) {
+                    u16 h0, l0, h1, l1;
+                    split_fmt<FMT>(x[i][(2 * e) * KT + tap] * scale, h0, l0);
+                    split_fmt<FMT>(x[i][(2 * e + 1) * KT + tap] * scale, h1, l1);
+                    h[e] = h0 | ((uint32_t)h1 << 16);
+                    l[e] = l0 | ((uint32_t)l1 << 16);
+                }
+                *(uint4*)(j.A_hi + idx) = make_uint4(h[0], h[1], h[2], h[3]);
+                if constexpr (!ONE) *(uint4*)(j.A_lo + idx) = make_uint4(l[0], l[1], l[2], l[3]);
+            }
         }
     }
 }
@@ -176,7 +194,7 @@
     __syncthreads();
     const int r = tid >> 4, cp = tid & 15;
     const int o = o0 + r;
-    if (o >= O) return;
+    if (o >= O || !j.A_hi) return;
     const int p = pack_dst_row(j, o);
     const float scale = s_scale[r];
     const float* vrow = j.v + (size_t)o * n;
@@ -193,7 +211,7 @@
 
 template <class FMT = T2sFmt, bool ONE = false>
 __global__ __launch_bounds__(256) void pack_table_kernel(const PackJob* __restrict__ jobs, int n_jobs) {
-    __shared__ float s_scale[16];
+    __shared__ float s_red[4][16];
     const long blk = blockIdx.x;
     int lo = 0, hi = n_jobs - 1;
     while (lo < hi) {
@@ -203,9 +221,11 @@
     const PackJob j = jobs[lo];
     const int o0 = (int)(blk - j.row_start) * 16;
     const int nchunk = ((int)j.Cin + 31) >> 5;
-    if (nchunk <= PACK_MAX_CHUNKS && !((int)j.Cin & 1) && j.Kt == 3) pack_rows_regs<3, FMT, ONE>(j, o0);
-    else if (nchunk <= PACK_MAX_CHUNKS && !((int)j.Cin & 1) && j.Kt == 1) pack_rows_regs<1, FMT, ONE>(j, o0);
-    else pack_rows_two_pass<FMT, ONE>(j, o0, s_scale);
+    const uintptr_t ptrs = (uintptr_t)j.v | (uintptr_t)j.A_hi | (ONE || !j.A_hi ? 0 : (uintptr_t)j.A_lo);
+    const bool wide = nchunk <= PACK_MAX_CHUNKS && !(((int)j.Cin | (int)j.koff | (int)j.Cin_pad) & 7) && !(ptrs & 15);
+    if (wide && j.Kt == 3) pack_rows_wide<3, FMT, ONE>(j, o0, s_red);
+    else if (wide && j.Kt == 1) pack_rows_wide<1, FMT, ONE>(j, o0, s_red);
+    else pack_rows_two_pass<FMT, ONE>(j, o0, s_red[0]);
 }
 hipError_t t2s_launch_pack_table(const PackJob* jobs, int n_jobs, long total_groups, hipStream_t stream, bool h16) {
     if (h16) hipLaunchKernelGGL((pack_table_kernel<T2sFmtF16, true>), dim3((unsigned)total_groups), dim3(256), 0, stream, jobs, n_jobs);
@@ -628,51 +648,58 @@
         for (int i = 0; i < n; ++i)
             for (int j = 0; j < n; ++j) inv_out[i * n + j] = (float)a[i][n + j];
 }
-static __device__ __forceinline__ void small_logdet_one(const SmallMatJob& j, float scale, double (*a)[32]) {
-    const int n = (int)j.n;
-    for (int i = 0; i < n; ++i)
-        for (int c = 0; c < n; ++c) {
-            a[i][c] = j.W[i * n + c];
-            a[i][n + c] = (i == c) ? 1.0 : 0.0;
-        }
+static __device__ __forceinline__ void small_logdet_one(const SmallMatJob& j, float scale) {
+    const int n = (int)j.n, q = threadIdx.x & 63;
+    double col[16];
+#pragma unroll
+    for (int i = 0; i < 16; ++i) {
+        col[i] = 0.0;
+        if (i < n && q < n) col[i] = j.W[i * n + q];
+        else if (i < n && q == n + i) col[i] = 1.0;
+    }
     double logabs = 0.0;
     int sign = 1;
-    for (int c = 0; c < n; ++c) {
+#pragma unroll
+    for (int c = 0; c < 16; ++c) {
+        if (c >= n) break;
         int piv = c;
-        double best = fabs(a[c][c]);
-        for (int r = c + 1; r < n; ++r)
-            if (fabs(a[r][c]) > best) { best = fabs(a[r][c]); piv = r; }
+        double best = fabs(col[c]);
+#pragma unroll
+        for (int r = c + 1; r < 16; ++r)
+            if (r < n && fabs(col[r]) > best) { best = fabs(col[r]); piv = r; }
+        piv = __shfl(piv, c, 64);
         if (piv != c) {
-            for (int q = 0; q < 2 * n; ++q) { double tmp = a[c][q]; a[c][q] = a[piv][q]; a[piv][q] = tmp; }
+#pragma unroll
+            for (int r = c + 1; r < 16; ++r)
+                if (r == piv) { const double tmp = col[c]; col[c] = col[r]; col[r] = tmp; }
             sign = -sign;
         }
-        const double d = a[c][c];
+        const double d = __shfl(col[c], c, 64);
         if (d < 0) sign = -sign;
         logabs += log(fabs(d));
         const double inv = 1.0 / d;
-        for (int q = 0; q < 2 * n; ++q) a[c][q] *= inv;
-        for (int r = 0; r < n; ++r) {
-            if (r == c) continue;
-            const double f = a[r][c];
+        col[c] *= inv;
+#pragma unroll
+        for (int r = 0; r < 16; ++r) {
+            if (r == c || r >= n) continue;
+            const double f = __shfl(col[r], c, 64);
             if (f == 0.0) continue;
-            for (int q = 0; q < 2 * n; ++q) a[r][q] -= f * a[c][q];
-        }
-    }
-    if (j.logdet_out) *j.logdet_out = sign > 0 ? (float)(logabs * (double)scale) : __builtin_nanf("");
-    if (j.inv_out)
-        for (int i = 0; i < n; ++i)
-            for (int c = 0; c < n; ++c) j.inv_out[i * n + c] = (float)a[i][n + c];
-}
-__global__ void small_logdet_batch_kernel(const SmallMatJob* jobs, float scale) {
-    __shared__ double a[16][32];
-    if (threadIdx.x != 0) return;
-    small_logdet_one(jobs[blockIdx.x], scale, a);
+            col[r] -= f * col[c];
+        }
+    }
+    if (j.logdet_out && q == 0) *j.logdet_out = sign > 0 ? (float)(logabs * (double)scale) : __builtin_nanf("");
+    if (j.inv_out && q >= n && q < 2 * n) {
+#pragma unroll
+        for (int i = 0; i < 16; ++i)
+            if (i < n) j.inv_out[i * n + (q - n)] = (float)col[i];
+    }
+}
+__global__ __launch_bounds__(64) void small_logdet_batch_kernel(const SmallMatJob* jobs, float scale) {
+    small_logdet_one(jobs[blockIdx.x], scale);
 }
 struct SmallMatJobs16 { SmallMatJob j[16]; };
-__global__ void small_logdet_batch_val_kernel(const SmallMatJobs16 jobs, float scale) {
-    __shared__ double a[16][32];
-    if (threadIdx.x != 0) return;
-    small_logdet_one(jobs.j[blockIdx.x], scale, a);
+__global__ __launch_bounds__(64) void small_logdet_batch_val_kernel(const SmallMatJobs16 jobs, float scale) {
+    small_logdet_one(jobs.j[blockIdx.x], scale);
 }
 hipError_t t2s_launch_small_logdet_batch(const SmallMatJob* jobs, int n_jobs, float scale, hipStream_t stream) {
     hipLaunchKernelGGL(small_logdet_batch_kernel, dim3(n_jobs), dim3(64), 0, stream, jobs, scale);
@@ -995,10 +1022,12 @@
     return hipGetLastError();
 }
 
-__global__ __launch_bounds__(256) void startfold_weights_kernel(const float* __restrict__ v, const float* __restrict__ g,
-                                                                const float* __restrict__ w_start,
-                                                                const float* __restrict__ b_start, int C, int nh, int Kt,
-                                                                int Mpad, int nwc, u16* A_hi, u16* A_lo) {
+template <bool TABLE>
+static __device__ __forceinline__ void startfold_weights_body(const float* __restrict__ v, const float* __restrict__ g,
+                                                              const float* __restrict__ w_start, const float* __restrict__ v_s,
+                                                              const float* __restrict__ g_s, float* __restrict__ w_out,
+                                                              const float* __restrict__ b_start, int C, int nh, int Kt,
+                                                              int Mpad, int nwc, u16* A_hi, u16* A_lo) {
     extern __shared__ float s_sf[];
     const int tid = threadIdx.x, wave = tid >> 6, lane = tid & 63, nwaves = blockDim.x >> 6;
     const int nw = nh + 1, n = C * Kt, O = 2 * C;
@@ -1025,7 +1054,22 @@
         for (int k = 0; k < 8; ++k)
             xr[k] = (vec && v0 + k * 256 < n) ? *(const float4*)(vrow + v0 + k * 256) : make_float4(0.f, 0.f, 0.f, 0.f);
 #pragma unroll
-        for (int k = 0; k < 8; ++k) wr[k] = w0 + k * bd < nws ? w_start[w0 + k * bd] : 0.f;
+        for (int k = 0; k < 8; ++k) {
+            const int i = w0 + k * bd;
+            if constexpr (TABLE) {
+                wr[k] = 0.f;
+                if (i < nws) {
+                    const int c = i / nh;
+                    float sq = 0.f;
+                    for (int kk = 0; kk < nh; ++kk) sq += v_s[c * nh + kk] * v_s[c * nh + kk];
+                    const float s = g_s ? g_s[c] / sqrtf(sq) : 1.f;
+                    wr[k] = v_s[i] * s;
+                    if (blockIdx.x == 0) w_out[i] = wr[k];
+                }
+            } else {
+                wr[k] = i < nws ? w_start[i] : 0.f;
+            }
+        }
 #pragma unroll
         for (int k = 0; k < 2; ++k) br[k] = b0 + k * bd < C ? b_start[b0 + k * bd] : 0.f;
 #pragma unroll
@@ -1072,13 +1116,47 @@
         A[((size_t)wc * Mpad + p) * 32 + col] = half ? l : h;
     }
 }
-hipError_t t2s_launch_startfold_weights(const float* v, const float* g, const float* w_start, const float* b_start, int C,
-                                        int n_half, int taps, int Mpad, int nwc, u16* A_hi, u16* A_lo, hipStream_t stream) {
+__global__ __launch_bounds__(256) void startfold_weights_kernel(const float* __restrict__ v, const float* __restrict__ g,
+                                                                const float* __restrict__ w_start,
+                                                                const float* __restrict__ b_start, int C, int nh, int Kt,
+                                                                int Mpad, int nwc, u16* A_hi, u16* A_lo) {
+    startfold_weights_body<false>(v, g, w_start, nullptr, nullptr, nullptr, b_start, C, nh, Kt, Mpad, nwc, A_hi, A_lo);
+}
+struct StartFoldJobs16 { StartFoldJob j[16]; };
+__global__ __launch_bounds__(256) void startfold_weights_table_kernel(const StartFoldJobs16 jobs, int C, int Kt, int Mpad, int nwc) {
+    const StartFoldJob& j = jobs.j[blockIdx.y];
+    startfold_weights_body<true>(j.v_in, j.g_in, nullptr, j.v_start, j.g_start, j.w_start, j.b_start, C, (int)j.n_half, Kt, Mpad,
+                                 nwc, j.A_hi, j.A_lo);
+}
+static int startfold_rows(int C, int n_half, int taps, size_t* lds_bytes) {
     const size_t wb = (size_t)((C * (n_half + 1) + 3) & ~3), row = (size_t)((C * taps + 3) & ~3);
     int rows = 4;
     while (rows > 1 && (wb + rows * row) * sizeof(float) > 65536) rows >>= 1;
-    hipLaunchKernelGGL(startfold_weights_kernel, dim3((2 * C + rows - 1) / rows), dim3(64 * rows),
-                       (wb + rows * row) * sizeof(float), stream, v, g, w_start, b_start, C, n_half, taps, Mpad, nwc, A_hi, A_lo);
+    *lds_bytes = (wb + rows * row) * sizeof(float);
+    return rows;
+}
+hipError_t t2s_launch_startfold_weights_table(const StartFoldJob* host_jobs, int n_jobs, int C, int taps, int Mpad, int nwc,
+                                              hipStream_t stream) {
+    if (n_jobs > 16) return hipErrorInvalidValue;
+    StartFoldJobs16 v;
+    memset(&v, 0, sizeof(v));
+    int nh_max = 0;
+    for (int i = 0; i < n_jobs; ++i) {
+        v.j[i] = host_jobs[i];
+        nh_max = (int)host_jobs[i].n_half > nh_max ? (int)host_jobs[i].n_half : nh_max;
+    }
+    size_t lds;
+    const int rows = startfold_rows(C, nh_max, taps, &lds);
+    hipLaunchKernelGGL(startfold_weights_table_kernel, dim3((2 * C + rows - 1) / rows, n_jobs), dim3(64 * rows), lds, stream, v, C,
+                       taps, Mpad, nwc);
+    return hipGetLastError();
+}
+hipError_t t2s_launch_startfold_weights(const float* v, const float* g, const float* w_start, const float* b_start, int C,
+                                        int n_half, int taps, int Mpad, int nwc, u16* A_hi, u16* A_lo, hipStream_t stream) {
+    size_t lds;
+    const int rows = startfold_rows(C, n_half, taps, &lds);
+    hipLaunchKernelGGL(startfold_weights_kernel, dim3((2 * C + rows - 1) / rows), dim3(64 * rows), lds, stream, v, g, w_start,
+                       b_start, C, n_half, taps, Mpad, nwc, A_hi, A_lo);
     return hipGetLastError();
 }
 
diff --git a/text2speech_amd/glow.py b/text2speech_amd/glow.py
--- a/text2speech_amd/glow.py
+++ b/text2speech_amd/glow.py
@@ -250,7 +250,7 @@
 
     def _pack(self, plan, device, force=False, flow_events=None):
         return plan._replace(pk=self.pack_weights(device, force=force, flow_events=flow_events, res_pair8=True,
-                                                  start_fold=plan.path.start_fold, h16=plan.h16))
+                                                  start_fold=plan.path.start_fold, h16=plan.h16, end_fold=True))
 
     def _stream(self, name, device):
         key = (name, str(device))
@@ -258,10 +258,10 @@
             self._streams[key] = torch.cuda.Stream(device=device)
         return self._streams[key]
 
-    def pack_weights(self, device, force=True, flow_events=None, res_pair8=False, start_fold=False, h16=False):
+    def pack_weights(self, device, force=True, flow_events=None, res_pair8=False, start_fold=False, h16=False, end_fold=False):
         assert not (h16 and (start_fold or flow_events is not None))
         res_pair8 = bool(res_pair8) and self.geom()["C"] % 32 == 0
-        key = tuple(p._version for p in self.m.parameters()) + (str(device), res_pair8, start_fold)
+        key = tuple(p._version for p in self.m.parameters()) + (str(device), res_pair8, start_fold, end_fold)
         slot = "packed16" if h16 else "packed"
         pk = getattr(self, slot)
         if (h16 or not force) and pk is not None and getattr(self, slot + "_key") == key:
@@ -269,7 +269,7 @@
         if pk is None or pk["device"] != device:
             pk = dict(flows=self._alloc_planes(device, h16), device=device, h16=h16)
             setattr(self, slot, pk)
-        srcs = self._pack_jobs(pk, res_pair8, start_fold)
+        srcs = self._pack_jobs(pk, res_pair8, start_fold, end_fold)
         fsrcs = self._fold_jobs(pk)
         starts = self._launch_pack(pk, start_fold, flow_events)
         setattr(self, slot + "_key", key)
@@ -340,7 +340,7 @@
                               A0h=bf16_only(*a0), A0l=bf16_only(*a0), w_inv=None))
         return flows
 
-    def _pack_jobs(self, pk, res_pair8, start_fold):
+    def _pack_jobs(self, pk, res_pair8, start_fold, end_fold=False):
         m, g = self.m, self.geom()
         C, nl, ks = g["C"], g["nl"], g["ks"]
         srcs = []
@@ -366,12 +366,20 @@
                     specs[k].append((t[4], t[5], None, None, ly["A1h"], ly["A1l"], None, 2 * C, g["n_cond"], 1, 1, C, g["Mpad1"],
                                      ks * g["Cpad"], g["Spad"], ly["s_cond"]))
                 p8 = res_pair8 and i < nl - 1
-                specs[k].append((t[6], t[7], t[8], None, ly["A2h"], ly["A2l"], ly["b2"], t[6].size(0), C, 1, 2 if p8 else 0,
-                                 C if p8 else 0, ly["Mpad2"], 0, g["Cpad"], ly["s_rs"]))
-        ptr_key = tuple(0 if t is None else t.data_ptr() for t in srcs) + (res_pair8, start_fold)
+                res_spec = lambda r0, O, planes: (
+                    (t[6], 4 * r0 * C), None if t[7] is None else (t[7], 4 * r0), t[8] if planes else None, None,
+                    ly["A2h"] if planes else None, ly["A2l"] if planes else None, ly["b2"] if planes else None, O, C, 1,
+                    2 if p8 else 0, C if p8 else 0, ly["Mpad2"], 0, g["Cpad"], (ly["s_rs"], 4 * r0))
+                if not end_fold:
+                    specs[k].append(res_spec(0, t[6].size(0), True))
+                elif i < nl - 1:
+                    specs[k] += [res_spec(0, C, True), res_spec(C, C, False)]
+                else:
+                    specs[k].append(res_spec(0, C, False))
+        ptr_key = tuple(0 if t is None else t.data_ptr() for t in srcs) + (res_pair8, start_fold, end_fold)
         if pk.get("job_key") != ptr_key:
             rows, flow_rows, flow_jobs = [], [], []
-            dp = lambda t: 0 if t is None else t.data_ptr()
+            dp = lambda t: 0 if t is None else t[0].data_ptr() + t[1] if isinstance(t, tuple) else t.data_ptr()
             for fspecs in specs:
                 row_start = 0
                 flow_jobs.append((len(rows), len(fspecs)))
@@ -414,27 +422,44 @@
         st = _lib.current_stream()
         jobs_ptr, fold_ptr = pk["jobs"].data_ptr(), pk["fold_jobs"].data_ptr()
         pack, endfold = _entry_point("pack", pk["h16"]), _entry_point("endfold", pk["h16"])
-        starts = []
+        starts, start_vg = [], []
+        for wn in m.WN:
+            v, gg = _vg(wn.start)
+            start_vg.append((_f32c(v), None if gg is None else _f32c(gg)))
+            starts += start_vg[-1]
+        if start_fold:
+            dp = lambda t: 0 if t is None else t.data_ptr()
+            rows = []
+            for k, wn in enumerate(m.WN):
+                fl = pk["flows"][k]
+                v0, g0 = _vg(wn.in_layers[0])
+                v0, g0, b_start = _f32c(v0), (None if g0 is None else _f32c(g0)), _f32c(wn.start.bias)
+                starts += [v0, g0, b_start]
+                rows.append([dp(v0), dp(g0), dp(start_vg[k][0]), dp(start_vg[k][1]), dp(b_start), dp(fl["w_start"]),
+                             dp(fl["A0h"]), dp(fl["A0l"]), fl["n_half"]])
+
+        def startfold_table(sub):
+            for k0 in range(0, len(sub), 16):
+                table = torch.tensor(sub[k0:k0 + 16], dtype=torch.int64)
+                _lib.call("t2s_wg_startfold_weights_table", ctypes.c_void_p(table.data_ptr()), table.size(0), C, ks, g["Mpad1"],
+                          g["nwc"], st)
+        if start_fold:
+            startfold_table(rows[:1])
         for k, wn in enumerate(m.WN):
             fl = pk["flows"][k]
             j0, nj = pk["flow_jobs"][k]
             _lib.call(pack, _lib.c_vp(jobs_ptr + j0 * 19 * 8), nj, pk["flow_rows"][k], st)
             _lib.call(endfold, _lib.c_vp(fold_ptr + k * nl * 8 * 8), nl, C, st)
-            v, gg = _vg(wn.start)
-            v, gg = _f32c(v), (None if gg is None else _f32c(gg))
-            starts += [v, gg]
-            _lib.call("t2s_weightnorm_small", _lib.ptr(v), _lib.ptr(gg), C, fl["n_half"], _lib.ptr(fl["w_start"]), st)
-            if start_fold:
-                v0, g0 = _vg(wn.in_layers[0])
-                v0, g0, b_start = _f32c(v0), (None if g0 is None else _f32c(g0)), _f32c(wn.start.bias)
-                starts += [v0, g0, b_start]
-                _lib.call("t2s_wg_startfold_weights", _lib.ptr(v0), _lib.ptr(g0), _lib.ptr(fl["w_start"]),
-                          _lib.ptr(b_start), C, fl["n_half"], ks, g["Mpad1"], g["nwc"], _lib.ptr(fl["A0h"]), _lib.ptr(fl["A0l"]), st)
+            if not start_fold:
+                v, gg = start_vg[k]
+                _lib.call("t2s_weightnorm_small", _lib.ptr(v), _lib.ptr(gg), C, fl["n_half"], _lib.ptr(fl["w_start"]), st)
             fl["w_inv"] = None
             if flow_events is not None:
                 ev = torch.cuda.Event()
                 ev.record()
                 flow_events.append(ev)
+            if start_fold and k == 0:
+                startfold_table(rows[1:])
         return starts
 
     def compose_geom(self):
@@ -671,14 +696,14 @@
         side.wait_stream(main)
         with torch.cuda.stream(side):
             st2 = _lib.current_stream()
+            if use_val:
+                _lib.call("t2s_small_logdet_inv_batch_host", ctypes.c_void_p(jobs.data_ptr()), m.n_flows, float(B * L), st2)
+            else:
+                _lib.call("t2s_small_logdet_inv_batch", _lib.ptr(jobs), m.n_flows, float(B * L), st2)
             _lib.call("t2s_wg_audio_squeeze", _lib.ptr(audio32), _lib.ptr(z), B, T, G, L, 0, st2)
             self._upsample(mel, B, L, w, plan)
             ev_inputs = torch.cuda.Event()
             ev_inputs.record()
-            if use_val:
-                _lib.call("t2s_small_logdet_inv_batch_host", ctypes.c_void_p(jobs.data_ptr()), m.n_flows, float(B * L), st2)
-            else:
-                _lib.call("t2s_small_logdet_inv_batch", _lib.ptr(jobs), m.n_flows, float(B * L), st2)
         pack_s = self._stream("pack", dev)
         pack_events = []
         pack_s.wait_stream(main)
```
